# YuvalNirkin/hyperseg

Measured on AMD Instinct MI355X. Metric: frames/sec @ bs=1 HyperSeg-M 1024x512, higher is better.
Workload: dtype f32 storage and accumulation; level-4 inverted residual products as 3-term f16 splits (f32-class: 1.3e-7 of sum|a||b|; exact_f32 beside it)

## Files before the change

### hyperseg_amd/_hip.py

```python
import ctypes as C
import os
import types

import torch

_LIB_PATH = os.environ.get('HS_HIP_LIB') or os.path.join(os.path.dirname(os.path.abspath(__file__)), 'lib',
                                                         'libhyperseg_hip.so')

ACT_NONE, ACT_RELU, ACT_RELU6, ACT_SWISH = 0, 1, 2, 3
PAD_MODES = {'zeros': 0, 'reflect': 1, 'replicate': 2, 'circular': 3}
PREV_NONE, PREV_SAME, PREV_BILINEAR = 0, 1, 2

_STATUS = {-1: 'bad argument', -2: 'feature map does not tile into the weight grid (H % fh or W % fw != 0)',
           -3: 'unsupported shape', -4: 'tile does not fit the LDS'}


class HipLibraryError(RuntimeError):
    pass


class StageInputC(C.Structure):
    _fields_ = [('skip', C.c_void_p), ('prev', C.c_void_p),
                ('batch', C.c_int32), ('H', C.c_int32), ('W', C.c_int32),
                ('c_skip', C.c_int32), ('c_prev', C.c_int32),
# ... 33 lines not shown


class TtaPassC(C.Structure):
    _fields_ = [('x', C.c_void_p), ('Hi', C.c_int32), ('Wi', C.c_int32), ('Hm', C.c_int32), ('Wm', C.c_int32),
                ('flipped', C.c_int32), ('entry', C.c_int32)]


STATUS = 'hs_status'
i32, i64, vp = C.c_int32, C.c_int64, C.c_void_p
SIGNATURES = {
    'hs_version': ([], C.c_int),
    'hs_build_info': ([], C.c_char_p),
    'hs_signal2weights_fwd': ([vp, i32, i32, i32, i32, i32, i32, i32, vp, i32, i32, vp, i64, vp], STATUS),
    'hs_signal2weights_multi_fwd': ([vp, i32, i32, i32, i32, C.POINTER(S2wLayerC), i32, vp], STATUS),
    'hs_s2w_pack_floats': ([i32, i32, i32], C.c_int64),
    'hs_s2w_pack_fwd': ([vp, i32, i32, i32, vp, vp], STATUS),
    'hs_bank_pack_fwd': ([vp, i32, i32, i32, i32, i32, i32, vp, i64, vp], STATUS),
    'hs_bn_fold_fwd': ([vp, vp, vp, vp, C.c_float, i32, vp, vp, vp], STATUS),
    'hs_patch_conv_fwd': ([C.POINTER(StageInputC), i32, i32, vp, i64, i32, i32, i32, i32, i32,
                           C.POINTER(EpilogueC), vp, vp], STATUS),
    'hs_patch_conv_s2w_fwd': ([C.POINTER(StageInputC), i32, i32, vp, i64, i32, i32, C.POINTER(EpilogueC), vp,
                               vp, i32, i32, i32, i32, C.POINTER(S2wLayerC), i32, vp], STATUS),
    'hs_k1_chain_workspace': ([i32, i32, i32, C.POINTER(K1LevelC), i32], C.c_int64),
    'hs_k1_chain_fwd': ([i32, i32, i32, C.POINTER(K1LevelC), i32, vp, vp, vp], STATUS),
    'hs_decoder_chain_workspace': ([i32, i32, i32, C.POINTER(K1LevelC), i32, C.POINTER(ChainIrLevelC)], C.c_int64),
    'hs_decoder_chain_fwd': ([i32, i32, i32, C.POINTER(K1LevelC), i32, C.POINTER(ChainIrLevelC), vp, vp, vp], STATUS),
    'hs_meta_conv_fwd': ([vp, i32, i32, i32, i32, vp, i64] + [i32] * 13 + [C.POINTER(EpilogueC), vp, vp], STATUS),
    'hs_meta_conv_bwd': ([vp, i32, i32, i32, i32, vp, i64] + [i32] * 12 + [vp, vp, vp, i64, vp], STATUS),
    'hs_patch_conv_gen_fwd': ([C.POINTER(StageInputC), i32, i32, vp, i32, C.POINTER(S2wLayerC), i32,
                               C.POINTER(EpilogueC), vp, vp], STATUS),
    'hs_patch_ir_fwd': ([C.POINTER(StageInputC), i32, i32, vp, i64, i32, i32, C.POINTER(EpilogueC),
                         C.POINTER(EpilogueC), C.POINTER(EpilogueC), i32, i32, vp, vp], STATUS),
    'hs_patch_ir_v0_fwd': ([C.POINTER(StageInputC), i32, i32, vp, i64, i32, i32, C.POINTER(EpilogueC),
                            C.POINTER(EpilogueC), C.POINTER(EpilogueC), i32, vp, vp], STATUS),
    'hs_patch_ir_v0_ws_fwd': ([C.POINTER(StageInputC), i32, i32, vp, i64, i32, i32, C.POINTER(EpilogueC),
                               C.POINTER(EpilogueC), C.POINTER(EpilogueC), i32, vp, i64, vp, vp], STATUS),
    'hs_patch_ir_v0_workspace': ([C.POINTER(StageInputC), i32, i32, i32, i32], C.c_int64),
    'hs_halo_tiles_fwd': ([i32, vp, i32, i32, i32, i32, i32, i32, vp, i32, vp], STATUS),
    'hs_halo_tiles_bwd': ([i32, vp, i32, i32, i32, i32, i32, i32, vp, i32, vp], STATUS),
    'hs_tile_interior_fwd': ([i32, vp, i32, i32, i32, i32, i32, i32, vp, vp], STATUS),
    'hs_tile_interior_bwd': ([i32, vp, i32, i32, i32, i32, i32, i32, vp, vp], STATUS),
    'hs_dw_tiles_fwd': ([i32, vp, vp, i64, i32, i32, i32, i32, i32, i32, vp, i32, vp], STATUS),
    'hs_dw_tiles_bwd_in': ([i32, vp, vp, i64, i32, i32, i32, i32, i32, i32, vp, i32, vp], STATUS),
    'hs_dw_tiles_bwd_w': ([i32, vp, vp, i32, i32, i32, i32, i32, i32, vp, i64, i32, vp], STATUS),
    'hs_bank_unpack_fwd': ([vp, i64, i32, i32, i32, i32, i32, i32, vp, vp], STATUS),
    'hs_upsample_bilinear_bwd': ([vp, i64, i32, i32, i32, i32, i32, i32, vp, vp], STATUS),
    'hs_upsample_bilinear_bf16_fwd': ([vp, i32, i32, i32, i32, i32, i32, vp, vp], STATUS),
    'hs_upsample_bilinear_f16_fwd': ([vp, i32, i32, i32, i32, i32, i32, vp, vp], STATUS),
    'hs_upsample_bilinear_typed_bwd': ([i32, vp, i64, i32, i32, i32, i32, i32, i32, vp, vp], STATUS),
    'hs_bn_train_workspace': ([i32], C.c_int64),
    'hs_bn_train_stats_fwd': ([i32, vp, i32, i32, i64, vp, vp], STATUS),
    'hs_dw_tiles_bn_fwd': ([i32, vp, vp, vp, vp, vp, vp, C.c_float, C.c_float, i32, vp, vp, vp, vp, i64, i32, i32, i32, i32, i32, i32, vp, i32, vp], STATUS),
    'hs_dw_tiles_bn_bwd_w': ([i32, vp, vp, vp, vp, vp, vp, i32, i32, i32, i32, i32, i32, i32, vp, i64, i32, vp], STATUS),
    'hs_s2w_train_fwd': ([vp, i32, i32, i32, i32, C.POINTER(S2wTrainLayerC), i32, vp], STATUS),
    'hs_s2w_train_workspace': ([i32, i32, i32, C.POINTER(S2wTrainLayerC), i32], C.c_int64),
    'hs_s2w_train_bwd': ([vp, i32, i32, i32, i32, C.POINTER(S2wTrainLayerC), i32, vp, vp, i64, vp], STATUS),
    'hs_cross_entropy_fwd': ([vp, vp, i32, i32, i64, i64, vp, vp], STATUS),
    'hs_cross_entropy_bwd': ([vp, vp, i32, i32, i64, i64, vp, vp, vp], STATUS),
    'hs_cross_entropy_typed_fwd': ([i32, vp, vp, i32, i32, i64, i64, vp, vp], STATUS),
    'hs_cross_entropy_typed_bwd': ([i32, vp, vp, i32, i32, i64, i64, vp, vp, vp], STATUS),
    'hs_bootstrapped_ce_fwd': ([i32, vp, vp, i32, i32, i64, i64, i32, C.c_float, vp, vp, vp, vp, vp], STATUS),
    'hs_bootstrapped_ce_bwd': ([i32, vp, vp, i32, i32, i64, i64, vp, vp, vp, vp, vp], STATUS),
    'hs_cross_entropy_weighted_fwd': ([i32, vp, vp, vp, i32, i32, i64, i64, vp, vp], STATUS),
    'hs_cross_entropy_weighted_bwd': ([i32, vp, vp, vp, i32, i32, i64, i64, vp, vp, vp], STATUS),
    'hs_bootstrapped_ce_weighted_fwd': ([i32, vp, vp, vp, i32, i32, i64, i64, i32, C.c_float, vp, vp, vp, vp, vp], STATUS),
    'hs_bootstrapped_ce_weighted_bwd': ([i32, vp, vp, vp, i32, i32, i64, i64, vp, vp, vp, vp, vp], STATUS),
    'hs_bn_act_train_fwd': ([i32, vp, i32, i32, i64, vp, vp, vp, vp, C.c_float, C.c_float, i32, vp, vp, vp, vp, vp, vp], STATUS),
    'hs_bn_act_train_bwd': ([i32, vp, vp, i32, i32, i64, vp, vp, vp, vp, C.c_float, i32, vp, vp, vp, vp, vp], STATUS),
    'hs_dw_tiles_bn_bwd_in_partials': ([i32, i32, i32, i32, i32], C.c_int64),
    'hs_dw_tiles_bn_bwd_in': ([i32, vp, vp, i64, vp, vp, vp, vp, vp, i32, i32, i32, i32, i32, i32, i32, vp, vp, i32, vp], STATUS),
    'hs_bn_act_train_bwd_apply': ([i32, vp, vp, i32, i32, i64, vp, vp, vp, vp, i32, vp, i64, vp, vp, vp, vp], STATUS),
    'hs_bootstrap_mean_workspace': ([], C.c_int64),
    'hs_bootstrap_mean_fwd': ([vp, i32, i32, C.c_float, vp, vp, vp], STATUS),
    'hs_bootstrap_mean_bwd': ([vp, i32, vp, vp, vp, vp], STATUS),
    'hs_bootstrap_mean_batched_fwd': ([vp, i32, i32, i32, C.c_float, vp, vp, vp], STATUS),
    'hs_bootstrap_mean_batched_bwd': ([vp, i32, i32, vp, vp, vp, vp], STATUS),
    'hs_patch_ir_route': ([C.POINTER(StageInputC), i32, i32, i32, i32, i32, i32], C.c_int),
    'hs_patch_ir_form': ([C.POINTER(StageInputC), i32, i32, i64, i32, i32, i32, i32, i32, i32, C.POINTER(C.c_int32)], C.c_int),
    'hs_patch_ir_v0_route': ([C.POINTER(StageInputC), i32, i32, i64, i32, i32, i32, i32, C.POINTER(C.c_int32)], C.c_int),
    'hs_patch_conv_route': ([C.POINTER(StageInputC), i32, i32, i64] + [i32] * 10 + [C.POINTER(C.c_int32)], C.c_int),
    'hs_ir_tile_map': ([i32, i32, i32, C.POINTER(i32), C.POINTER(i32), C.POINTER(i32), i32], STATUS),
    'hs_upsample_bilinear_fwd': ([vp, i32, i32, i32, i32, i32, i32, vp, vp], STATUS),
    'hs_upsample_argmax_fwd': ([vp, i32, i32, i32, i32, i32, i32, vp, vp], STATUS),
    'hs_eval_max_classes': ([], C.c_int),
    'hs_upsample_confusion_fwd': ([vp, i32, i32, i32, i32, i32, i32, vp, i32, i32, i32, vp, vp, vp], STATUS),
    'hs_confusion_fwd': ([vp, i32, vp, i32, i32, i64, i32, i32, vp, vp], STATUS),
    'hs_upsample2_confusion_fwd': ([vp, i32, i32, i32, i32, i32, i32, i32, i32, vp, i32, i32, i32, vp, vp, vp], STATUS),
    'hs_tta_merge_fwd': ([C.POINTER(TtaPassC), i32, i32, i32, i32, vp, i32, i32, i32, i32, i32, vp, vp, vp, vp], STATUS),
    'hs_cross_entropy_score_fwd': ([i32, vp, vp, i32, i32, i64, i64, vp, i32, i32, vp, vp, vp], STATUS),
    'hs_upsample_ce_confusion_fwd': ([vp, i32, i32, i32, i32, i32, i32, vp, i32, i64, vp, i32, i32, vp, vp, vp], STATUS),
    'hs_cross_entropy_score_weighted_fwd': ([i32, vp, vp, vp, i32, i32, i64, i64, vp, i32, i32, vp, vp, vp], STATUS),
    'hs_upsample_ce_confusion_weighted_fwd': ([vp, i32, i32, i32, i32, i32, i32, vp, i32, vp, i64, vp, i32, i32, vp, vp, vp], STATUS),
    'hs_upsample2_ce_confusion_fwd': ([vp, i32, i32, i32, i32, i32, i32, i32, i32, vp, i32, i64, vp, i32, i32, vp, vp, vp], STATUS),
    'hs_upsample2_ce_confusion_weighted_fwd': ([vp, i32, i32, i32, i32, i32, i32, i32, i32, vp, i32, vp, i64, vp, i32, i32, vp, vp, vp], STATUS),
    'hs_stage_input_fwd': ([C.POINTER(StageInputC), vp, vp], STATUS),
    'hs_stage_input_typed_fwd': ([C.POINTER(StageInputC), i32, i32, vp, vp], STATUS),
    'hs_patch_conv_bwd_input': ([vp, vp, i64, i32, i32, i32, i32, i32, i32, i32, i32, i32, i32, i32, vp, vp], STATUS),
    'hs_patch_conv_bwd_weight': ([vp, vp, i32, i32, i32, i32, i32, i32, i32, i32, i32, i32, i32, vp, i64, vp], STATUS),
    'hs_patch_conv_bwd_route': ([i32, i32, i32, i32, i64] + [i32] * 11 + [C.POINTER(C.c_int32), C.POINTER(C.c_int32)], STATUS),
    'hs_patch_conv_plain_fwd': ([i32, vp, vp, i64, i32, i32, i32, i32, i32, i32, i32, i32, i32, i32, i32, vp, vp], STATUS),
    'hs_patch_conv_plain_bwd_in': ([i32, vp, vp, i64, i32, i32, i32, i32, i32, i32, i32, i32, i32, i32, i32, vp, vp], STATUS),
    'hs_patch_conv_plain_bwd_w': ([i32, vp, vp, i32, i32, i32, i32, i32, i32, i32, i32, i32, i32, i32, vp, i64, vp], STATUS),
    'hs_depthwise_conv_fwd': ([vp, i32, i32, i32, i32, vp, i32, i32, i32, i32, i32, i32, vp, vp, i32, vp, vp, vp, vp, vp], STATUS),
    'hs_pointwise_conv_fwd': ([vp, i32, i32, i32, vp, i32, vp, vp, vp, i32, vp, vp, vp], STATUS),
    'hs_affine_act_fwd': ([vp, i32, i32, i32, vp, vp, i32, vp, vp, vp], STATUS),
    'hs_patch_conv_bn_fwd': ([i32, vp, vp, vp, vp, vp, vp, C.c_float, C.c_float, i32, vp, vp, vp, vp, i64, i32, i32, i32, i32, i32, i32, i32, vp, vp], STATUS),
    'hs_patch_conv_bn_bwd_w': ([i32, vp, vp, vp, vp, vp, vp, i32, i32, i32, i32, i32, i32, i32, i32, vp, i64, vp], STATUS),
    'hs_bootstrap_mean_of_batch_fwd': ([vp, i32, i32, i32, C.c_float, vp, vp, vp, vp], STATUS),
    'hs_bootstrap_mean_of_batch_bwd': ([vp, i32, i32, vp, vp, vp, vp], STATUS),
    'hs_adam_blocks': ([vp, i32], C.c_int64),
    'hs_adam_step': ([vp, vp, vp, vp, vp, i32, vp, C.c_float, C.c_double, C.c_double, C.c_float, C.c_float, i32, i32, vp, vp], STATUS),
    'hs_adam_step_amp': ([vp, vp, vp, vp, vp, i32, vp, C.c_float, C.c_double, C.c_double, C.c_float, C.c_float, i32, i32, vp, vp, vp, vp], STATUS),
    'hs_depthwise_pool_blocks': ([i32, i32], C.c_int),
    'hs_depthwise_conv_se_fwd': ([vp, i32, i32, i32, i32, vp, i32, i32, i32, i32, i32, i32, vp, vp, i32, vp, vp, vp, C.POINTER(SeTailC), vp], STATUS),
    'hs_mbconv_expand_dw_se_fwd': ([vp, i32, i32, i32, i32, vp, i32, vp, vp, vp, i32, i32, i32, i32, i32, i32, vp, vp, vp, C.POINTER(SeTailC), vp], STATUS),
    'hs_se_tail_workspace': ([i32, i32, i32, i32, i64], C.c_int64),
    'hs_se_tail_tails': ([i32, i32, i32, i64], C.c_int),
    'hs_mbconv_se_workgroups': ([i32, i32, i32, i32, i32, i32], C.c_int64),
    'hs_stem_conv_fwd': ([vp, i32, i32, i32, i32, vp, i32, i32, i32, i32, i32, vp, vp, vp, vp], STATUS),
    'hs_mbconv_tiles': ([i32, i32, i32, i32], C.c_int),
    'hs_stem_dw_fwd': ([vp, i32, i32, i32, vp, i32, vp, vp, i32, i32, i32, i32, vp, i32, i32, i32, vp, vp, vp, vp, vp], STATUS),
    'hs_image_ingest_fwd': ([vp, i32, i32, i32, i32, i32, vp, vp, vp], STATUS),
    'hs_stem_dw_u8_fwd': ([vp, i32, vp, i32, i32, i32, vp, i32, vp, vp, i32, i32, i32, i32, vp, i32, i32, i32, vp, vp, vp, vp, vp], STATUS),
    'hs_overlay_fwd': ([vp, vp, i32, i32, i32, i32, vp, i32, i32, vp, vp], STATUS),
    'hs_upsample_overlay_fwd': ([vp, i32, i32, i32, i32, i32, i32, vp, i32, vp, i32, i32, vp, vp, vp], STATUS),
    'hs_upsample2_overlay_fwd': ([vp, i32, i32, i32, i32, i32, i32, i32, i32, vp, i32, vp, i32, i32, vp, vp, vp], STATUS),
    'hs_confidence_fwd': ([vp, i32, i32, i32, i32, i32, C.c_float, i32, vp, vp, vp], STATUS),
    'hs_upsample_confidence_fwd': ([vp, i32, i32, i32, i32, i32, i32, i32, C.c_float, i32, vp, vp, vp], STATUS),
    'hs_upsample2_confidence_fwd': ([vp, i32, i32, i32, i32, i32, i32, i32, i32, i32, C.c_float, i32, vp, vp, vp], STATUS),
    'hs_frame_resize_fwd': ([vp, i32, i32, i32, i32, vp, vp, i32, i32, vp, vp, i32, i32, i32, i32, i32, i32, i32, C.c_uint32, vp, vp, vp], STATUS),
    'hs_label_resize_fwd': ([vp, i32, i32, i32, i32, vp, i32, vp, i32, i32, i32, i32, i32, i32, i32, vp, i32, vp], STATUS),
    'hs_resize_tables_fwd': ([vp, i32, i32, i32, i32, i32, i32, i32, vp, vp, vp, vp, vp], STATUS),
    'hs_frame_resize_batch_fwd': ([vp, i32, i32, i32, i32, vp, vp, vp, vp, i32, i32, i32, C.c_uint32, vp, vp, vp], STATUS),
    'hs_label_resize_batch_fwd': ([vp, i32, i32, i32, i32, vp, vp, vp, i32, i32, i32, vp, i32, vp], STATUS),
    'hs_label_encode_fwd': ([vp, i32, i32, i32, i32, vp, i32, i32, i32, vp, i32, vp], STATUS),
    'hs_label_resize_coded_fwd': ([vp, i32, i32, i32, i32, vp, i32, vp, i32, i32, i32, i32, i32, i32, i32, vp, i32, i32, i32, vp, i32, vp], STATUS),
    'hs_label_resize_batch_coded_fwd': ([vp, i32, i32, i32, i32, vp, vp, vp, i32, i32, i32, vp, i32, i32, i32, vp, i32, vp], STATUS),
    'hs_color_jitter_fwd': ([vp, i32, i32, i32, i32, vp, vp, vp, vp, vp], STATUS),
    'hs_gaussian_blur_fwd': ([vp, i32, i32, i32, i32, vp, vp, vp, vp, vp, vp], STATUS),
    'hs_frame_rotate_fwd': ([vp, i32, i32, i32, i32, vp, i32, i32, C.c_uint32, C.c_uint32, vp, vp, vp], STATUS),
    'hs_label_rotate_fwd': ([vp, i32, i32, i32, i32, vp, i32, i32, i32, i32, vp, i32, vp], STATUS),
    'hs_resize_tables_ragged_fwd': ([vp, i32, i32, i32, i32, i32, i32, i32, vp, vp, vp, vp, vp], STATUS),
    'hs_color_jitter_ragged_fwd': ([vp, i32, i32, i32, i32, vp, vp, vp, vp, vp], STATUS),
    'hs_frame_resize_ragged_fwd': ([vp, i32, i32, i32, i32, vp, vp, vp, vp, i32, i32, i32, vp, vp], STATUS),
    'hs_label_resize_ragged_fwd': ([vp, i32, i32, i32, i32, vp, vp, vp, i32, i32, vp, vp], STATUS),
    'hs_frame_rotate_ragged_fwd': ([vp, i32, i32, i32, i32, vp, vp, vp, i32, i32, C.c_uint32, C.c_uint32, vp, vp, vp], STATUS),
    'hs_label_rotate_ragged_fwd': ([vp, i32, i32, i32, vp, vp, vp, i32, i32, i32, i32, vp, i32, vp], STATUS),
    'hs_mbconv_expand_dw_fwd': ([vp, i32, i32, i32, i32, vp, i32, vp, vp, vp, i32, i32, i32, i32, i32, i32, vp, vp, vp, vp, vp], STATUS),
    'hs_se_gate_fwd': ([vp, i32, i32, i32, C.c_float, vp, vp, i32, vp, vp, vp, vp, vp, i32, vp, vp, vp], STATUS),
    'hs_gemm_split_kp': ([i32], C.c_int),
    'hs_gemm_split_fwd': ([vp, vp, vp, vp, vp, i32, vp, vp, i32, i32, i32, i32, i32, vp], STATUS),
    'hs_gemm_split_se_fwd': ([vp, vp, vp, i32, C.c_float, vp, vp, i32, vp, vp, vp, vp, i32, vp, vp, i32, i32, i32, i32, i32, vp, vp, vp], STATUS),
    'hs_gemm_split_se_route': ([i32] * 6, C.c_int),
    'hs_gemm_split_conv2x2_fwd': ([vp, vp, vp, vp, i32, vp, vp, i32, i32, i32, i32, i32, i32, vp], STATUS),
    'hs_gemm_split_up2_fwd': ([vp, vp, vp, vp, i32, vp, i32, i32, i32, i32, i32, i32, vp], STATUS),
    'hs_depthwise_route': ([i32] * 11, C.c_int),
    'hs_mbconv_route': ([i32] * 11, C.c_int),
    'hs_stem_dw_route': ([i32] * 9, C.c_int),
    'hs_stem_route': ([i32] * 3, C.c_int),
    'hs_se_gate_route': ([i32] * 5, C.c_int),
    'hs_pointwise_route': ([i32] * 5, C.c_int),
    'hs_pooled_shift_fwd': ([vp, i32, C.c_float, vp, vp, vp, i32, i32, vp], STATUS),
}
EXPORTS = list(SIGNATURES)


def check(status, what):
    if status == 0:
        return
    if status < 0:
        raise HipLibraryError(f'{what}: {_STATUS.get(status, status)}')
    raise HipLibraryError(f'{what}: HIP launch failed with hipError_t {status}')


def _raise_unless_ok(status, fn, args):
    if status:
        check(status, fn.__name__)
    return status


def _load():
    if not os.path.exists(_LIB_PATH):
        raise HipLibraryError(
            f'{_LIB_PATH} is missing: build it with `python -m hyperseg_amd.build` (hipcc, gfx950). '
            'hyperseg_amd has no fallback path.')
    lib = C.CDLL(_LIB_PATH)
    run = types.SimpleNamespace()
    for name, (argtypes, returns) in SIGNATURES.items():
        fn = getattr(lib, name)
        fn.argtypes, fn.restype = argtypes, C.c_int if returns is STATUS else returns
        if returns is STATUS:
            checked = lib[name]
            checked.argtypes, checked.restype, checked.errcheck = argtypes, C.c_int, _raise_unless_ok
            setattr(run, name, checked)
    if lib.hs_version() != 1:
        raise HipLibraryError(f'ABI mismatch: library reports version {lib.hs_version()}, binding expects 1')
    return lib, run


lib, run = _load()


def ptr(t):
    return None if t is None else t.data_ptr()


def dev_ptr(t, name='tensor', dtype=torch.float32):
    if t is None:
        return None
    if not isinstance(t, torch.Tensor):
        raise TypeError(f'{name} must be a torch.Tensor')
    if not t.is_cuda:
        raise HipLibraryError(f'{name} is on {t.device}: the HyperSeg decoder path runs on an MI355X only '
                              '(hyperseg_amd has no CPU fallback)')
    if t.dtype != dtype:
        raise HipLibraryError(f'{name} must be {dtype}, got {t.dtype}')
    if not t.is_contiguous():
        raise HipLibraryError(f'{name} must be contiguous')
    return t.data_ptr()


class _NullScope:
    def __enter__(self):
        return None

    def __exit__(self, *exc):
        return False


_NULL_SCOPE = _NullScope()


def device_scope(device):
    if device.index is None or device.index == torch.cuda.current_device():
        return _NULL_SCOPE
    return torch.cuda.device(device)


def stream_ptr(device=None):
    return torch.cuda.current_stream(device).cuda_stream
```

### hyperseg_amd/csrc/hs_encoder.hip

```cpp
#include "hs_common.h"
#include "hs_se_tail.h"

namespace hs {

template <int K, int S, int PL, bool TILE, bool SET>
__global__ __launch_bounds__(256)
void depthwise_conv_kernel(const float* __restrict__ x, const float* __restrict__ w, const float* __restrict__ scale,
                           const float* __restrict__ shift, float* __restrict__ y, int C, int H, int W, int Ho, int Wo,
                           int pad_t, int pad_l, int act, float* __restrict__ pool_partial,
                           const float* __restrict__ in_scale, const float* __restrict__ in_shift, int nplanes, SeTail se) {
    const int plane = blockIdx.y + blockIdx.z * gridDim.y;
    if (plane >= nplanes) return;
    const int c = plane % C;
    unsigned se_gen = 0u;
    if constexpr (SET) se_gen = se.ws ? se_tag(se, plane / C) : 0u;
    const bool pre = in_scale != nullptr;
    float isc = 1.0f, ish = 0.0f;
    if constexpr (TILE) {
        if (pre) { isc = in_scale[c]; ish = in_shift[c]; }
    }
    const int wq = (Wo + 3) >> 2;
    const int q = blockIdx.x * blockDim.x + threadIdx.x;
    const bool live = q < Ho * wq;
    float psum = 0.0f;
// ... 463 lines not shown
                                 const hs_se_tail* se_in, void* stream) {
    if ((in_scale != nullptr) != (in_shift != nullptr)) return HS_ERR_BAD_ARG;
    if (!x || !w || !y || batch <= 0 || channels <= 0 || H <= 0 || W <= 0 || Ho <= 0 || Wo <= 0) return HS_ERR_BAD_ARG;
    if (pad_t < 0 || pad_l < 0 || (scale && !shift)) return HS_ERR_BAD_ARG;
    const long nplanes = (long)batch * channels;
    if (nplanes > 65535L * 65535L) return HS_ERR_UNSUPPORTED;
    const int quads = Ho * ((Wo + 3) / 4);
    const int threads = depthwise_threads(Ho, Wo);
    const int gy = nplanes > 65535 ? 32768 : (int)nplanes;
    dim3 grid((quads + threads - 1) / threads, gy, (unsigned)((nplanes + gy - 1) / gy));
    hipStream_t s = (hipStream_t)stream;
    SeTail se{};
    if (se_in) {
        const int st = make_se_tail(se_in, batch, channels, (int)grid.x, (long)channels * grid.x, Ho * Wo, se);
        if (st != HS_OK) return st;
    }
    const size_t se_lds = se_in ? (size_t)se_lds_floats(se.Csq) * sizeof(float) : 0;
#define HS_DW_(KK, SS, PP, SETV) hipLaunchKernelGGL((depthwise_conv_kernel<KK, SS, PP, false, SETV>), grid, dim3(threads), se_lds, s, x, w, scale, shift, \
                                             y, channels, H, W, Ho, Wo, pad_t, pad_l, act, pool_partial, in_scale, in_shift, (int)nplanes, se)
#define HS_DW(KK, SS, PP) do { if (se_in) HS_DW_(KK, SS, PP, true); else HS_DW_(KK, SS, PP, false); } while (0)
    const int route = depthwise_route(nplanes, k, stride, pad_l, W, Ho, Wo, (((size_t)x) & 15) == 0, in_scale != nullptr);
    if (route < 0) return route;
    if ((route >> 8) == HS_DW_FORM_TILED) {
        const size_t tile_lds = depthwise_tile_lds(k, stride, Wo);
        const size_t lds = tile_lds > se_lds ? tile_lds : se_lds;
#define HS_DWT_(KK, SS, SETV) hipLaunchKernelGGL((depthwise_conv_kernel<KK, SS, -1, true, SETV>), grid, dim3(threads), lds, s, x, w, scale, shift, y, \
                                          channels, H, W, Ho, Wo, pad_t, pad_l, act, pool_partial, in_scale, in_shift, (int)nplanes, se)
#define HS_DWT(KK, SS) do { if (se_in) HS_DWT_(KK, SS, true); else HS_DWT_(KK, SS, false); } while (0)
        if (k == 3 && stride == 1) HS_DWT(3, 1); else if (k == 3) HS_DWT(3, 2); else if (stride == 1) HS_DWT(5, 1); else HS_DWT(5, 2);
#undef HS_DWT
#undef HS_DWT_
        return launch_status();
    }
    switch (route) {
        case HS_DW_ROUTE(HS_DW_FORM_VECTOR, 3, 1, 1): HS_DW(3, 1, 1); break;
        case HS_DW_ROUTE(HS_DW_FORM_GENERIC, 3, 1, 0): HS_DW(3, 1, -1); break;
        case HS_DW_ROUTE(HS_DW_FORM_VECTOR, 3, 2, 0): HS_DW(3, 2, 0); break;
        case HS_DW_ROUTE(HS_DW_FORM_VECTOR, 3, 2, 1): HS_DW(3, 2, 1); break;
        case HS_DW_ROUTE(HS_DW_FORM_GENERIC, 3, 2, 0): HS_DW(3, 2, -1); break;
        case HS_DW_ROUTE(HS_DW_FORM_VECTOR, 5, 1, 2): HS_DW(5, 1, 2); break;
        case HS_DW_ROUTE(HS_DW_FORM_GENERIC, 5, 1, 0): HS_DW(5, 1, -1); break;
        case HS_DW_ROUTE(HS_DW_FORM_VECTOR, 5, 2, 1): HS_DW(5, 2, 1); break;
        case HS_DW_ROUTE(HS_DW_FORM_VECTOR, 5, 2, 2): HS_DW(5, 2, 2); break;
        case HS_DW_ROUTE(HS_DW_FORM_GENERIC, 5, 2, 0): HS_DW(5, 2, -1); break;
        default: return HS_ERR_UNSUPPORTED;
    }
#undef HS_DW
#undef HS_DW_
    return launch_status();
}

extern "C" int hs_depthwise_route(int32_t batch, int32_t channels, int32_t H, int32_t W, int32_t k, int32_t stride, int32_t pad_l,
                                  int32_t Ho, int32_t Wo, int32_t x_aligned16, int32_t prologue) {
    if (batch <= 0 || channels <= 0 || H <= 0 || W <= 0 || Ho <= 0 || Wo <= 0 || pad_l < 0) return HS_ERR_BAD_ARG;
    if ((long)batch * channels > 65535L * 65535L) return HS_ERR_UNSUPPORTED;
    return depthwise_route((long)batch * channels, k, stride, pad_l, W, Ho, Wo, x_aligned16 != 0, prologue != 0);
}

extern "C" int hs_depthwise_conv_fwd(const float* x, int32_t batch, int32_t channels, int32_t H, int32_t W,
                                     const float* w, int32_t k, int32_t stride, int32_t pad_t, int32_t pad_l,
                                     int32_t Ho, int32_t Wo, const float* scale, const float* shift, int32_t act,
                                     float* y, float* pool_partial, const float* in_scale, const float* in_shift,
                                     void* stream) {
    return depthwise_conv_launch(x, batch, channels, H, W, w, k, stride, pad_t, pad_l, Ho, Wo, scale, shift, act, y, pool_partial,
                                 in_scale, in_shift, nullptr, stream);
}

extern "C" int hs_depthwise_conv_se_fwd(const float* x, int32_t batch, int32_t channels, int32_t H, int32_t W,
                                        const float* w, int32_t k, int32_t stride, int32_t pad_t, int32_t pad_l,
                                        int32_t Ho, int32_t Wo, const float* scale, const float* shift, int32_t act,
                                        float* y, const float* in_scale, const float* in_shift, const hs_se_tail* se,
                                        void* stream) {
    if (!se) return HS_ERR_BAD_ARG;
    return depthwise_conv_launch(x, batch, channels, H, W, w, k, stride, pad_t, pad_l, Ho, Wo, scale, shift, act, y, nullptr,
                                 in_scale, in_shift, se, stream);
}

extern "C" int64_t hs_se_tail_workspace(int32_t batch, int32_t channels, int32_t c_squeezed, int32_t nblk, int64_t wgs_per_batch) {
    int T, L;
    if (batch <= 0 || !se_tail_plan(channels, c_squeezed, nblk, wgs_per_batch, T, L)) return 0;
    SeTail t{};
    t.B = batch; t.C = channels; t.Csq = c_squeezed; t.nblk = nblk; t.T = T; t.L = L;
    return (int64_t)(se_ws_words(t) * sizeof(se_u64));
}

extern "C" int hs_se_tail_tails(int32_t channels, int32_t c_squeezed, int32_t nblk, int64_t wgs_per_batch) {
    int T, L;
    return se_tail_plan(channels, c_squeezed, nblk, wgs_per_batch, T, L) ? T : 0;
}

extern "C" int hs_depthwise_pool_blocks(int32_t Ho, int32_t Wo) {
    const int quads = Ho * ((Wo + 3) / 4);
    const int threads = quads >= 256 ? 256 : ((quads + 63) / 64) * 64;
    return (quads + threads - 1) / threads;
}

static int se_early_fold(int nblk) { return nblk <= 256 ? 1 : (nblk <= 512 ? 2 : 4); }

static int se_gate_route(int channels, int nblk, int c_squeezed, bool proj, bool aligned16) {
    const long units = (long)channels * ((nblk & 3) == 0 ? nblk >> 2 : nblk);
    if ((channels & 3) == 0 && channels <= 768 && c_squeezed <= SEF_MAX_CSQ && units <= 2048) return HS_SE_ROUTE_FUSED;
    static const bool off = [] { const char* e = getenv("HS_SE_EARLY"); return e && atoi(e) == 0; }();
    const int fold = se_early_fold(nblk);
    if (!off && !proj && (channels & 3) == 0 && channels * fold <= 4 * SEE_MAX_IT && c_squeezed <= 8 && (nblk & (4 * fold - 1)) == 0 &&
        nblk <= 1024 && aligned16) return HS_SE_ROUTE_EARLY;
    if (HS_SE_FUSED_WIDE && (channels & 3) == 0 && channels <= 256 && c_squeezed <= SEF_MAX_CSQ && units <= 6144) return HS_SE_ROUTE_FUSED_WIDE;
    return HS_SE_ROUTE_TWO_LAUNCH;
}

extern "C" int hs_se_gate_route(int32_t channels, int32_t nblk, int32_t c_squeezed, int32_t with_w_proj, int32_t aligned16) {
    if (channels <= 0 || nblk <= 0 || c_squeezed <= 0) return HS_ERR_BAD_ARG;
    if (c_squeezed > 65535) return HS_ERR_UNSUPPORTED;
    return se_gate_route(channels, nblk, c_squeezed, with_w_proj != 0, aligned16 != 0);
}

extern "C" int hs_se_gate_fwd(const float* partial, int32_t batch, int32_t channels, int32_t nblk, float inv_hw,
                              const float* w_reduce, const float* b_reduce, int32_t c_squeezed, const float* w_expand,
                              const float* b_expand, float* squeezed, float* gate, const float* w_proj, int32_t c_out,
                              const float* out_scale, float* w_scaled, void* stream) {
    if (!partial || !w_reduce || !b_reduce || !w_expand || !b_expand || !squeezed || !gate || batch <= 0 || channels <= 0 ||
        nblk <= 0 || c_squeezed <= 0) return HS_ERR_BAD_ARG;
    if ((w_proj != nullptr) != (w_scaled != nullptr) || (w_proj && c_out <= 0) || (out_scale && !w_proj)) return HS_ERR_BAD_ARG;
    if (batch > 65535 || c_squeezed > 65535) return HS_ERR_UNSUPPORTED;
    hipStream_t s = (hipStream_t)stream;
    const int row_groups = w_proj ? (c_out + 63) / 64 : 1;
    const int route = se_gate_route(channels, nblk, c_squeezed, w_proj != nullptr, (((size_t)partial | (size_t)w_reduce) & 15) == 0);
    if (route == HS_SE_ROUTE_FUSED) {
        hipLaunchKernelGGL((se_gate_fused_kernel<8, 3>), dim3((channels + 63) / 64, batch, row_groups), dim3(256), 0, s, partial, nblk,
                           inv_hw, w_reduce, b_reduce, w_expand, b_expand, channels, c_squeezed, squeezed, gate, w_proj, c_out,
                           out_scale, w_scaled);
        return launch_status();
    }
    if (route == HS_SE_ROUTE_EARLY) {
        const int fold = se_early_fold(nblk);
        hipLaunchKernelGGL(se_gate_early_kernel, dim3(1, batch), dim3(256), 0, s, partial, nblk / fold, inv_hw, w_reduce, b_reduce, w_expand,
                           b_expand, channels * fold, c_squeezed, squeezed, gate, fold);
        return launch_status();
    }
    if (route == HS_SE_ROUTE_FUSED_WIDE) {
        hipLaunchKernelGGL((se_gate_fused_kernel<24, 1>), dim3((channels + 63) / 64, batch, row_groups), dim3(256), 0, s, partial, nblk,
                           inv_hw, w_reduce, b_reduce, w_expand, b_expand, channels, c_squeezed, squeezed, gate, w_proj, c_out,
                           out_scale, w_scaled);
        return launch_status();
    }
    hipLaunchKernelGGL(se_squeeze_kernel, dim3(c_squeezed, batch), dim3(256), 0, s, partial, nblk, inv_hw, w_reduce,
                       b_reduce, channels, c_squeezed, squeezed);
    int st = launch_status();
    if (st != HS_OK) return st;
    hipLaunchKernelGGL(se_excite_kernel, dim3((channels + 63) / 64, batch, row_groups), dim3(256), 0, s, squeezed, w_expand,
                       b_expand, channels, c_squeezed, gate, w_proj, c_out, out_scale, w_scaled);
    return launch_status();
}

namespace hs {

using f32x4 = __attribute__((ext_vector_type(4))) float;

template <int NB, int NT, bool VEC = false>
__global__ __launch_bounds__(256)
void pointwise_conv_kernel(const float* __restrict__ x, const float* __restrict__ w, const float* __restrict__ gate,
                           const float* __restrict__ scale, const float* __restrict__ shift,
                           const float* __restrict__ residual, float* __restrict__ y, int Cin, int Cout, int P, int act) {
    const int lane = threadIdx.x & 63, wave = threadIdx.x >> 6;
    const int lrow = lane & 15, lk = lane >> 4;
    const int b = blockIdx.z;
    const int o0 = blockIdx.y * 32;
    const int p0 = (blockIdx.x * 4 + wave) * (16 * NT);
    if (p0 >= P) return;
    const float* __restrict__ xb = x + (size_t)b * Cin * P;
    const float* __restrict__ gb = gate ? gate + (size_t)b * Cin : nullptr;
    f32x4 acc[2][NT];
#pragma unroll
    for (int m = 0; m < 2; ++m)
#pragma unroll
        for (int n = 0; n < NT; ++n) acc[m][n] = f32x4{0.f, 0.f, 0.f, 0.f};
    int orow[2]; bool ook[2];
#pragma unroll
    for (int m = 0; m < 2; ++m) { const int o = o0 + 16 * m + lrow; ook[m] = o < Cout; orow[m] = ook[m] ? o : Cout - 1; }
    int pcol[NT]; bool pok[NT];
#pragma unroll
    for (int n = 0; n < NT; ++n) { const int p = VEC ? p0 + 4 * lrow + n : p0 + 16 * n + lrow; pok[n] = p < P; pcol[n] = pok[n] ? p : P - 1; }
    static_assert(!VEC || NT == 4, "interleaved tiles: four pixels per lane");
    constexpr int KU = 4;
    float av[2][KU][2], bv[2][KU][NT];
    auto load_batch = [&](int i, float (&a)[KU][2], float (&bb)[KU][NT]) {
#pragma unroll
        for (int u = 0; u < KU; ++u) {
            const int k = i * 4 * KU + 4 * u + lk;
            const bool kok = k < Cin;
            const int kc = kok ? k : Cin - 1;
            const float g = (gb ? gb[kc] : 1.0f) * (kok ? 1.0f : 0.0f);
#pragma unroll
            for (int m = 0; m < 2; ++m) a[u][m] = w[(size_t)orow[m] * Cin + kc] * (ook[m] ? 1.0f : 0.0f);
            if constexpr (VEC) {
                const f32x4 v = *reinterpret_cast<const f32x4*>(xb + (size_t)kc * P + pcol[0]);
#pragma unroll
                for (int n = 0; n < NT; ++n) bb[u][n] = v[n] * g;
            } else {
#pragma unroll
                for (int n = 0; n < NT; ++n) bb[u][n] = xb[(size_t)kc * P + pcol[n]] * g;
            }
        }
    };
    load_batch(0, av[0], bv[0]);
    float scv[2][4], shv[2][4];
#pragma unroll
    for (int m = 0; m < 2; ++m)
#pragma unroll
        for (int r = 0; r < 4; ++r) {
            const int o = min(o0 + 16 * m + 4 * lk + r, Cout - 1);
            scv[m][r] = scale ? scale[o] : 1.0f;
            shv[m][r] = shift ? shift[o] : 0.0f;
        }
    float rv[2][4][NT];
    if (residual) {
#pragma unroll
        for (int m = 0; m < 2; ++m)
#pragma unroll
            for (int r = 0; r < 4; ++r) {
                const int o = min(o0 + 16 * m + 4 * lk + r, Cout - 1);
                if constexpr (VEC) {
                    const f32x4 v = *reinterpret_cast<const f32x4*>(residual + ((size_t)b * Cout + o) * P + pcol[0]);
#pragma unroll
                    for (int n = 0; n < NT; ++n) rv[m][r][n] = v[n];
                } else {
#pragma unroll
                    for (int n = 0; n < NT; ++n) rv[m][r][n] = residual[((size_t)b * Cout + o) * P + pcol[n]];
                }
            }
    } else {
#pragma unroll
        for (int m = 0; m < 2; ++m)
#pragma unroll
            for (int r = 0; r < 4; ++r)
#pragma unroll
                for (int n = 0; n < NT; ++n) rv[m][r][n] = 0.0f;
    }
#pragma unroll
    for (int i = 0; i < NB; ++i) {
        if (i + 1 < NB) load_batch(i + 1, av[(i + 1) & 1], bv[(i + 1) & 1]);
#pragma unroll
        for (int u = 0; u < KU; ++u)
#pragma unroll
            for (int m = 0; m < 2; ++m)
#pragma unroll
                for (int n = 0; n < NT; ++n)
                    acc[m][n] = __builtin_amdgcn_mfma_f32_16x16x4f32(av[i & 1][u][m], bv[i & 1][u][n], acc[m][n], 0, 0, 0);
    }
#pragma unroll
    for (int m = 0; m < 2; ++m)
#pragma unroll
        for (int r = 0; r < 4; ++r) {
            const int o = o0 + 16 * m + 4 * lk + r;
            if (o >= Cout) continue;
            float ov[NT];
#pragma unroll
            for (int n = 0; n < NT; ++n) {
                float v = fmaf(acc[m][n][r], scv[m][r], shv[m][r]);
                if (act == 3) v = swishf(v);
                else v = apply_act(v, act);
                ov[n] = v + rv[m][r][n];
            }
            if constexpr (VEC) {
                *reinterpret_cast<f32x4*>(y + ((size_t)b * Cout + o) * P + pcol[0]) = f32x4{ov[0], ov[1], ov[2], ov[3]};
            } else {
#pragma unroll
                for (int n = 0; n < NT; ++n)
                    if (pok[n]) y[((size_t)b * Cout + o) * P + pcol[n]] = ov[n];
            }
        }
}

template <int NB>
static int launch_pointwise(int nt, bool vec, dim3 grid, hipStream_t s, const float* x, const float* w, const float* gate,
                            const float* scale, const float* shift, const float* residual, float* y, int c_in, int c_out,
                            int pixels, int act) {
#define HS_PW(NT) hipLaunchKernelGGL((pointwise_conv_kernel<NB, NT>), grid, dim3(256), 0, s, x, w, gate, scale, shift, \
                                     residual, y, c_in, c_out, pixels, act)
    if (vec) hipLaunchKernelGGL((pointwise_conv_kernel<NB, 4, true>), grid, dim3(256), 0, s, x, w, gate, scale, shift, residual, y, c_in,
                                c_out, pixels, act);
    else if (nt == 4) HS_PW(4); else if (nt == 2) HS_PW(2); else HS_PW(1);
#undef HS_PW
    return launch_status();
}

}

static int pointwise_route(int batch, int c_in, int c_out, int pixels, bool aligned16) {
    if (batch > 65535 || (c_out + 31) / 32 > 65535) return HS_ERR_UNSUPPORTED;
    if (c_in > 128) return HS_ERR_UNSUPPORTED;
    const int mblocks = (c_out + 31) / 32;
    int nt = 4;
    while (nt > 1 && (long)((pixels + 64 * nt - 1) / (64 * nt)) * mblocks * batch < 512) nt >>= 1;
    static const bool vec_off = [] { const char* e = getenv("HS_PW_VEC"); return e && atoi(e) == 0; }();
    const bool vec = !vec_off && nt == 4 && (pixels & 63) == 0 && aligned16;
    const int nb = (c_in + 15) / 16;
    return HS_PW_ROUTE(nb, nt, vec ? 1 : 0);
}

extern "C" int hs_pointwise_route(int32_t batch, int32_t c_in, int32_t c_out, int32_t pixels, int32_t aligned16) {
    if (batch <= 0 || c_in <= 0 || c_out <= 0 || pixels <= 0) return HS_ERR_BAD_ARG;
    return pointwise_route(batch, c_in, c_out, pixels, aligned16 != 0);
}

extern "C" int hs_pointwise_conv_fwd(const float* x, int32_t batch, int32_t c_in, int32_t pixels, const float* w,
                                     int32_t c_out, const float* gate, const float* scale, const float* shift, int32_t act,
// ... 171 lines not shown
```

### hyperseg_amd/csrc/hs_gemm_split.hip

```cpp
#include "hs_common.h"
#include "hs_se_gate_phases.h"
#include <type_traits>

namespace hs {

using half8 = __attribute__((ext_vector_type(8))) _Float16;
using gs_f32x4 = __attribute__((ext_vector_type(4))) float;

__device__ __forceinline__ int gs_exp_of(float m) { return min(max(__float_as_int(m) >> 23, 27), 254); }
__device__ __forceinline__ float gs_scale_of(int eb) { return __int_as_float((268 - eb) << 23); }
__device__ __forceinline__ float gs_inv_scale_of(int eb) { return __int_as_float((eb - 14) << 23); }

struct GemmSplitArgs {
    const _Float16* __restrict__ wf;
    const float* __restrict__ w_inv;
    const float* __restrict__ gate; const float* __restrict__ x;
    const float* shift;
    const float* residual;
    float* y;
    int M, K, KST, N, act;
    int conv_wo;
    float* pool_partial;
    int up2_wo;
};

struct GemmSeArgs {
    const float* __restrict__ partial;
    const float* __restrict__ w1; const float* __restrict__ b1;
    const float* __restrict__ w2t; const float* __restrict__ b2;
    float* gate_out; float* squeezed_out;
    float inv_hw; int nblk, Csq;
};
template <bool SEG> struct GemmSeOperand {};
template <> struct GemmSeOperand<true> : GemmSeArgs {};

#ifndef HS_GS_NARROW_MAX_WG
#define HS_GS_NARROW_MAX_WG 128
#endif

#ifndef HS_GS_TALL_MIN_WG
#define HS_GS_TALL_MIN_WG 257
#endif

template <int KS, int NWV, bool FAST, int NS, int MT, int NCH, bool PATCH, bool SEG = false>
__global__ __launch_bounds__(64 * NWV)
void gemm_split_kernel(GemmSplitArgs a, GemmSeOperand<SEG> se) {
    static_assert(!SEG || (FAST && !PATCH && NCH == 1 && (NWV == 8 ? KS <= 3 : KS == 1)), "SEG: the project convolutions' forms only");
    extern __shared__ __attribute__((aligned(16))) float gs_red[];
    constexpr int nthr = 64 * NWV, nwv = NWV;
    constexpr int NP = 16 * NS, NR = 16 * MT, NE = NR * NP;
    const int tid = threadIdx.x, lane = tid & 63, wave = tid >> 6;
    const int lrow = lane & 15, kg = lane >> 4;
    const int n0 = blockIdx.x * NP, r0 = blockIdx.y * MT, b = blockIdx.z;
    const float* __restrict__ xb = a.x + (size_t)b * a.K * a.N;
    const float* __restrict__ gb = a.gate ? a.gate + (size_t)b * a.K : nullptr;
    float* yb = a.y + (size_t)b * a.M * a.N * (a.up2_wo > 0 ? 4 : 1);
    const float* rb = a.residual ? a.residual + (size_t)b * a.M * a.N : nullptr;
    const int rt_max = (a.M + 15) >> 4;

    using gs_f32x2 = __attribute__((ext_vector_type(2))) float;
    const int ncol0 = min(n0 + NS * lrow, a.N - (FAST && !PATCH && NS == 2 ? 2 : 1)), ncol1 = min(n0 + NS * lrow + 1, a.N - 1);
    float xv[NCH][NS][KS][8];
    if constexpr (PATCH) {
        const int oy = ncol0 / a.conv_wo, ox = ncol0 - oy * a.conv_wo;
        const float* __restrict__ win = xb + (size_t)(2 * oy) * (2 * a.conv_wo) + 2 * ox;
        const int cmax = (a.K >> 2) - 1;
#pragma unroll
        for (int c = 0; c < NCH; ++c)
#pragma unroll
            for (int s = 0; s < KS; ++s)
#pragma unroll
                for (int q = 0; q < 4; ++q) {
                    const int ch = min((((wave * NCH + c) * KS + s) * 32 + 8 * kg) / 4 + (q >> 1), cmax);
                    const float* src = win + (size_t)ch * (4 * a.N) + (q & 1) * (2 * a.conv_wo);
                    if constexpr (NS == 1) {
                        const gs_f32x2 v = *reinterpret_cast<const gs_f32x2*>(src);
                        xv[c][0][s][2 * q] = v[0]; xv[c][0][s][2 * q + 1] = v[1];
                    } else {
                        const gs_f32x4 v = *reinterpret_cast<const gs_f32x4*>(src);
                        xv[c][0][s][2 * q] = v[0]; xv[c][0][s][2 * q + 1] = v[1];
                        xv[c][1][s][2 * q] = v[2]; xv[c][1][s][2 * q + 1] = v[3];
                    }
                }
    } else {
#pragma unroll
        for (int c = 0; c < NCH; ++c)
#pragma unroll
            for (int s = 0; s < KS; ++s)
#pragma unroll
                for (int j = 0; j < 8; ++j) {
                    const int k = ((wave * NCH + c) * KS + s) * 32 + 8 * kg + j;
                    const int kc = min(k, a.K - 1);
                    if constexpr (NS == 1) {
                        xv[c][0][s][j] = xb[(size_t)kc * a.N + ncol0];
                    } else if constexpr (FAST) {
                        const gs_f32x2 v = *reinterpret_cast<const gs_f32x2*>(xb + (size_t)kc * a.N + ncol0);
                        xv[c][0][s][j] = v[0]; xv[c][1][s][j] = v[1];
                    } else {
                        xv[c][0][s][j] = xb[(size_t)kc * a.N + ncol0]; xv[c][1][s][j] = xb[(size_t)kc * a.N + ncol1];
                    }
                }
    }
    constexpr int NG = PATCH ? 1 : NCH;
    float gv[NG][KS][8];
    if constexpr (!PATCH) {
#pragma unroll
        for (int c = 0; c < NCH; ++c)
#pragma unroll
            for (int s = 0; s < KS; ++s) {
                const int k0 = ((wave * NCH + c) * KS + s) * 32 + 8 * kg;
                if constexpr (SEG) {
                } else if constexpr (FAST) {
                    const float* gp = gb ? gb + min(k0, a.K - 8) : a.w_inv;
                    const gs_f32x4 g0 = *reinterpret_cast<const gs_f32x4*>(gp), g1 = *reinterpret_cast<const gs_f32x4*>(gp + 4);
#pragma unroll
                    for (int j = 0; j < 4; ++j) { gv[c][s][j] = g0[j]; gv[c][s][4 + j] = g1[j]; }
                } else {
#pragma unroll
                    for (int j = 0; j < 8; ++j) gv[c][s][j] = gb ? gb[min(k0 + j, a.K - 1)] : 1.0f;
                }
            }
    }
    half8 ah[2][KS], al[2][KS];
    auto load_a = [&](int q) {
        const int rt = min(r0 + q % MT, rt_max - 1);
#pragma unroll
        for (int s = 0; s < KS; ++s) {
            const _Float16* blk = a.wf + ((size_t)(rt * a.KST + (wave * NCH + q / MT) * KS + s) * 2) * 512 + lane * 8;
            ah[q & 1][s] = *reinterpret_cast<const half8*>(blk);
            al[q & 1][s] = *reinterpret_cast<const half8*>(blk + 512);
        }
    };
    load_a(0);
    constexpr int TE = (NE + nthr - 1) / nthr;
    float wi[TE], sh[TE], yo[TE];
    auto load_tail = [&]() {
#pragma unroll
        for (int i = 0; i < TE; ++i) {
            const int e = min(tid + i * nthr, NE - 1);
            const int row = min(16 * r0 + e / NP, a.M - 1), col = min(n0 + (e & (NP - 1)), a.N - 1);
            wi[i] = a.w_inv[min(16 * r0 + e / NP, 16 * rt_max - 1)];
            sh[i] = a.shift ? a.shift[row] : 0.0f;
            yo[i] = rb ? rb[(size_t)row * a.N + col] : 0.0f;
        }
    };
    constexpr bool LATE_TAIL = KS * NCH >= 3;
    if constexpr (!LATE_TAIL) load_tail();
    constexpr int SE_PV = SEP_MAX_UNITS / nthr, SE_RW = SEP_MAX_CSQ / NWV, SE_W1U = NWV == 8 ? (KS < 3 ? KS : 3) : 1;
    constexpr int SE_CI = NWV == 8 && KS >= 3 ? 2 : 1;
    float4 se_pv[SE_PV], se_w1v[SE_RW][SE_W1U];
    float se_b1v[SE_RW], se_w2q[SE_CI][4][8], se_b2v[SE_CI];
    if constexpr (SEG) {
        se_load_units<nthr, SE_PV>(se.partial + (size_t)b * a.K * se.nblk, se.nblk, a.K, tid, se_pv);
        se_load_reduce<NWV, SE_RW, SE_W1U>(se.w1, se.b1, a.K, se.Csq, wave, lane, se_w1v, se_b1v);
#pragma unroll
        for (int ci = 0; ci < SE_CI; ++ci) se_load_expand(se.w2t, se.b2, a.K, se.Csq, min(tid + nthr * ci, a.K - 1), se_w2q[ci], se_b2v[ci]);
    }
    __builtin_amdgcn_sched_barrier(0);
    if constexpr (SEG) {
        float* mean_c = gs_red + SEP_MEAN; float* zs = gs_red + SEP_ZS; float* gate_s = gs_red + SEP_GATE;
        se_channel_means<nthr, SE_PV>(se_pv, se.nblk, a.K, se.inv_hw, tid, gs_red + SEP_PART, mean_c);
        se_squeeze_rows<NWV, SE_RW, SE_W1U>(se_w1v, se_b1v, mean_c, a.K, se.Csq, wave, lane, zs);
        __syncthreads();
        const bool first = blockIdx.x == 0 && blockIdx.y == 0;
        if (first && se.squeezed_out && tid < se.Csq) se.squeezed_out[(size_t)b * se.Csq + tid] = zs[tid];
#pragma unroll
        for (int ci = 0; ci < SE_CI; ++ci) {
            const int ch = tid + nthr * ci;
            const float g = se_channel_gate(se_w2q[ci], se_b2v[ci], zs, se.Csq);
            if (ch < a.K) {
                gate_s[ch] = g;
                if (first && se.gate_out) se.gate_out[(size_t)b * a.K + ch] = g;
            }
        }
        __syncthreads();
#pragma unroll
        for (int s = 0; s < KS; ++s) {
            const float* gp = gate_s + min((wave * KS + s) * 32 + 8 * kg, a.K - 8);
            const gs_f32x4 g0 = *reinterpret_cast<const gs_f32x4*>(gp), g1 = *reinterpret_cast<const gs_f32x4*>(gp + 4);
#pragma unroll
            for (int j = 0; j < 4; ++j) { gv[0][s][j] = g0[j]; gv[0][s][4 + j] = g1[j]; }
        }
        __syncthreads();
    }

    gs_f32x4 tot[MT][NS];
#pragma unroll
    for (int c = 0; c < NCH; ++c) {
        float invb[NS];
        half8 bh[NS][KS], bl[NS][KS];
#pragma unroll
        for (int t = 0; t < NS; ++t) {
            unsigned mx = 0;
#pragma unroll
            for (int s = 0; s < KS; ++s) {
                const int k0 = ((wave * NCH + c) * KS + s) * 32 + 8 * kg;
#pragma unroll
                for (int j = 0; j < 8; ++j) {
                    const float mk = (FAST || PATCH ? k0 : k0 + j) < a.K ? 1.0f : 0.0f;
                    float g = mk;
                    if constexpr (!PATCH) g = SEG || gb ? gv[c][s][j] * mk : mk;
                    xv[c][t][s][j] *= g;
                    mx = max(mx, __float_as_uint(xv[c][t][s][j]) & 0x7fffffffu);
                }
            }
            {
                auto r16 = __builtin_amdgcn_permlane16_swap(mx, mx, false, false);
                mx = max(r16[0], r16[1]);
                auto r32 = __builtin_amdgcn_permlane32_swap(mx, mx, false, false);
                mx = max(r32[0], r32[1]);
            }
            const int eb = gs_exp_of(__uint_as_float(mx));
            const float sc = gs_scale_of(eb);
            invb[t] = gs_inv_scale_of(eb);
#pragma unroll
            for (int s = 0; s < KS; ++s) {
                if constexpr (FAST || PATCH) {
                    unsigned hh[4], ll[4];
#pragma unroll
                    for (int j = 0; j < 4; ++j) {
                        asm("v_fma_mixlo_f16 %0, %2, %4, 0\n\t"
                            "v_fma_mixhi_f16 %0, %3, %4, 0\n\t"
                            "v_fma_mixlo_f16 %1, %2, %4, -%0 op_sel_hi:[0,0,1]\n\t"
                            "v_fma_mixhi_f16 %1, %3, %4, -%0 op_sel:[0,0,1] op_sel_hi:[0,0,1]"
                            : "=&v"(hh[j]), "=&v"(ll[j]) : "v"(xv[c][t][s][2 * j]), "v"(xv[c][t][s][2 * j + 1]), "v"(sc));
                    }
                    using gs_u32x4 = __attribute__((ext_vector_type(4))) unsigned;
                    bh[t][s] = __builtin_bit_cast(half8, gs_u32x4{hh[0], hh[1], hh[2], hh[3]});
                    bl[t][s] = __builtin_bit_cast(half8, gs_u32x4{ll[0], ll[1], ll[2], ll[3]});
                } else {
#pragma unroll
                    for (int j = 0; j < 8; ++j) {
                        const float v = xv[c][t][s][j] * sc;
                        const _Float16 hi = (_Float16)v;
                        bh[t][s][j] = hi;
                        bl[t][s][j] = (_Float16)(v - (float)hi);
                    }
                }
            }
        }
        if (c == 0) {
            load_a(1);
            if constexpr (LATE_TAIL) load_tail();
        }
        __builtin_amdgcn_sched_barrier(0);
#pragma unroll
        for (int mt = 0; mt < MT; ++mt) {
            const int q = c * MT + mt;
            gs_f32x4 acc[NS];
#pragma unroll
            for (int t = 0; t < NS; ++t) {
                acc[t] = gs_f32x4{0.f, 0.f, 0.f, 0.f};
#pragma unroll
                for (int s = 0; s < KS; ++s) {
                    acc[t] = __builtin_amdgcn_mfma_f32_16x16x32_f16(al[q & 1][s], bh[t][s], acc[t], 0, 0, 0);
                    acc[t] = __builtin_amdgcn_mfma_f32_16x16x32_f16(ah[q & 1][s], bl[t][s], acc[t], 0, 0, 0);
                    acc[t] = __builtin_amdgcn_mfma_f32_16x16x32_f16(ah[q & 1][s], bh[t][s], acc[t], 0, 0, 0);
                }
            }
            if (q + 2 < NCH * MT) { load_a(q + 2); __builtin_amdgcn_sched_barrier(0); }
#pragma unroll
            for (int t = 0; t < NS; ++t) {
#pragma unroll
                for (int r = 0; r < 4; ++r) {
                    const float v = c == 0 ? acc[t][r] * invb[t] : fmaf(acc[t][r], invb[t], tot[mt][t][r]);
                    if (c == NCH - 1) gs_red[(wave * NR + 16 * mt + 4 * kg + r) * NP + NS * lrow + t] = v;
                    else tot[mt][t][r] = v;
                }
            }
        }
    }
    __syncthreads();
    auto tail = [&](auto act_kind) {
        constexpr int ACT = decltype(act_kind)::value;
#pragma unroll
        for (int i = 0; i < TE; ++i) {
            const int e = tid + i * nthr;
            if (e < NE) {
                const int row = 16 * r0 + e / NP, col = n0 + (e & (NP - 1));
                float t = 0.0f;
#pragma unroll
                for (int w = 0; w < nwv; ++w) t += gs_red[w * NE + e];
                const bool live = row < a.M && col < a.N;
                float v = fmaf(t, wi[i], sh[i]);
                if constexpr (ACT == HS_ACT_SWISH) v = swishf(v);
                else if constexpr (ACT == HS_ACT_RELU) v = fmaxf(v, 0.0f);
                else if constexpr (ACT == HS_ACT_RELU6) v = fminf(fmaxf(v, 0.0f), 6.0f);
                v += yo[i];
                if (live) {
                    if (a.up2_wo > 0) {
                        const int oy = col / a.up2_wo, ox = col - oy * a.up2_wo;
                        float* dst = yb + (size_t)row * (4 * a.N) + (size_t)(2 * oy) * (2 * a.up2_wo) + 2 * ox;
                        *reinterpret_cast<gs_f32x2*>(dst) = gs_f32x2{v, v};
                        *reinterpret_cast<gs_f32x2*>(dst + 2 * a.up2_wo) = gs_f32x2{v, v};
                    } else {
                        yb[(size_t)row * a.N + col] = v;
                    }
                }
                if constexpr (NP == 16) {
                    if (a.pool_partial) {
                        const float rs = rowsum16(live ? v : 0.0f);
                        if ((e & 15) == 0 && row < a.M) a.pool_partial[((size_t)b * a.M + row) * gridDim.x + blockIdx.x] = rs;
                    }
                }
            }
        }
    };
    if (a.act == HS_ACT_SWISH) tail(std::integral_constant<int, HS_ACT_SWISH>{});
    else if (a.act == HS_ACT_NONE) tail(std::integral_constant<int, HS_ACT_NONE>{});
    else if (a.act == HS_ACT_RELU) tail(std::integral_constant<int, HS_ACT_RELU>{});
    else tail(std::integral_constant<int, HS_ACT_RELU6>{});
}

__global__ __launch_bounds__(256)
void pooled_shift_kernel(const float* __restrict__ partial, int nblk, float inv_p, const float* __restrict__ wb,
                         const float* __restrict__ shift, float* __restrict__ out, int M, int C) {
    extern __shared__ float ps_mean[];
    const int tid = threadIdx.x, lane = tid & 63, wave = tid >> 6;
    for (int c = tid; c < C; c += 256) {
        float t = 0.0f;
        for (int j = 0; j < nblk; ++j) t += partial[(size_t)c * nblk + j];
        ps_mean[c] = t * inv_p;
    }
    __syncthreads();
    const int r0 = 16 * blockIdx.x + 4 * wave;
    float acc[4] = {0.f, 0.f, 0.f, 0.f};
#pragma unroll 2
    for (int c = lane; c < C; c += 64) {
        const float m = ps_mean[c];
#pragma unroll
        for (int i = 0; i < 4; ++i) acc[i] = fmaf(wb[(size_t)min(r0 + i, M - 1) * C + c], m, acc[i]);
    }
#pragma unroll
    for (int i = 0; i < 4; ++i) {
        const float t = wave_sum64(acc[i]);
        if (lane == 0 && r0 + i < M) out[r0 + i] = shift[r0 + i] + t;
    }
}

static bool gemm_split_plan(int K, int& nwv, int& ks, int& nch) {
    const int steps = (K + 31) / 32;
    nwv = 2;
    while (nwv < 8 && nwv < steps) nwv *= 2;
    const int per = (steps + nwv - 1) / nwv;
    nch = per > 5 ? 2 : 1;
    ks = (steps + nwv * nch - 1) / (nwv * nch);
    return ks <= 5;
}

}

using namespace hs;

extern "C" int hs_gemm_split_kp(int32_t c_in) {
    int nwv, ks, nch;
    if (c_in <= 0 || !gemm_split_plan(c_in, nwv, ks, nch)) return HS_ERR_UNSUPPORTED;
    return nwv * nch * ks * 32;
}

struct GemmSplitPolicy {
    int nwv, ks, nch;
    bool narrow, tall, fast;
    dim3 grid;
    size_t lds;
};
static int gemm_split_policy(int batch, int c_out, int c_in, int kp, int pixels, GemmSplitPolicy& p) {
    if (!gemm_split_plan(c_in, p.nwv, p.ks, p.nch)) return HS_ERR_UNSUPPORTED;
    if (kp != p.nwv * p.nch * p.ks * 32 || (p.ks > 1 && p.nwv != 8)) return HS_ERR_BAD_ARG;
    if (batch > 65535 || (c_out + 31) / 32 > 65535) return HS_ERR_UNSUPPORTED;
    p.grid = dim3((pixels + 31) / 32, ((c_out + 15) / 16 + 1) / 2, batch);
    const size_t wgs = (size_t)p.grid.x * p.grid.y * p.grid.z;
    p.narrow = wgs <= HS_GS_NARROW_MAX_WG && pixels > 16;
    p.tall = wgs >= HS_GS_TALL_MIN_WG && c_out > 32;
    if (p.narrow) p.grid.x = (pixels + 15) / 16;
    if (p.tall) p.grid.y = ((c_out + 15) / 16 + 3) / 4;
    p.lds = (size_t)p.nwv * (p.narrow ? 512 : p.tall ? 2048 : 1024) * sizeof(float);
    p.fast = (c_in & 7) == 0 && (pixels & 1) == 0 && c_in >= 8;
    return HS_OK;
}

static int launch_gemm_split_plain(const void* w_frag, const float* w_inv, const float* gate, const float* x, const float* shift,
                                   int32_t act, const float* residual, float* y, int32_t batch, int32_t c_out, int32_t c_in,
                                   int32_t kp, int32_t pixels, int up2_wo, void* stream) {
    if (!w_frag || !w_inv || !x || !y || batch <= 0 || c_out <= 0 || c_in <= 0 || pixels <= 0) return HS_ERR_BAD_ARG;
    if (act < 0 || act > 3) return HS_ERR_BAD_ARG;
    GemmSplitPolicy pol;
    const int pst = gemm_split_policy(batch, c_out, c_in, kp, pixels, pol);
    if (pst != HS_OK) return pst;
    const int nwv = pol.nwv, ks = pol.ks, nch = pol.nch;
    const bool narrow = pol.narrow, tall = pol.tall, fast = pol.fast;
    dim3 grid = pol.grid;
    const size_t lds = pol.lds;
    GemmSplitArgs a{(const _Float16*)w_frag, w_inv, gate, x, shift, residual, y, c_out, c_in, kp / 32, pixels, act, 0, nullptr, up2_wo};
    hipStream_t s = (hipStream_t)stream;
#define HS_GS_(KSV, NWV, F) do { \
        if (narrow) hipLaunchKernelGGL((gemm_split_kernel<KSV, NWV, F, 1, 2, 1, false>), grid, dim3(64 * NWV), lds, s, a, GemmSeOperand<false>{}); \
        else if (tall) hipLaunchKernelGGL((gemm_split_kernel<KSV, NWV, F, 2, 4, 1, false>), grid, dim3(64 * NWV), lds, s, a, GemmSeOperand<false>{}); \
        else hipLaunchKernelGGL((gemm_split_kernel<KSV, NWV, F, 2, 2, 1, false>), grid, dim3(64 * NWV), lds, s, a, GemmSeOperand<false>{}); } while (0)
#define HS_GS(KSV, NWV) do { if (fast) HS_GS_(KSV, NWV, true); else HS_GS_(KSV, NWV, false); } while (0)
    if (nch == 2) {
        if (!fast || up2_wo > 0) return HS_ERR_UNSUPPORTED;
        grid.x = (pixels + 15) / 16; grid.y = ((c_out + 15) / 16 + 1) / 2;
        const size_t lds2 = (size_t)8 * 512 * sizeof(float);
#define HS_GS2(KSV) hipLaunchKernelGGL((gemm_split_kernel<KSV, 8, true, 1, 2, 2, false>), grid, dim3(512), lds2, s, a, GemmSeOperand<false>{})
        switch (ks) { case 3: HS_GS2(3); break; case 4: HS_GS2(4); break; case 5: HS_GS2(5); break; default: return HS_ERR_UNSUPPORTED; }
#undef HS_GS2
        return launch_status();
    }
    switch (ks) {
        case 1: if (nwv == 2) HS_GS(1, 2); else if (nwv == 4) HS_GS(1, 4); else HS_GS(1, 8); break;
        case 2: HS_GS(2, 8); break;
        case 3: HS_GS(3, 8); break;
        case 4: HS_GS(4, 8); break;
        default: HS_GS(5, 8); break;
    }
#undef HS_GS
#undef HS_GS_
    return launch_status();
}

static int gemm_split_se_route(int channels, int nblk, int c_squeezed, int c_out, int pixels, bool aligned16, int batch, GemmSplitPolicy& pol) {
    if (channels <= 0 || nblk <= 0 || c_squeezed <= 0 || c_out <= 0 || pixels <= 0 || batch <= 0) return HS_ERR_BAD_ARG;
    const int kp = hs_gemm_split_kp(channels);
    if (kp < 0) return HS_ERR_UNSUPPORTED;
    const int pst = gemm_split_policy(batch, c_out, channels, kp, pixels, pol);
    if (pst != HS_OK) return pst;
    if (hs_se_gate_route(channels, nblk, c_squeezed, 0, aligned16 ? 1 : 0) != HS_SE_ROUTE_FUSED) return HS_ERR_UNSUPPORTED;
    if (!aligned16 || !pol.fast || pol.nch != 1 || channels > SEP_MAX_C || c_squeezed > SEP_MAX_CSQ) return HS_ERR_UNSUPPORTED;
    if (pol.ks > (pol.nwv == 8 ? 3 : 1)) return HS_ERR_UNSUPPORTED;
    return HS_GSE_ROUTE(pol.ks, pol.nwv);
}

extern "C" int hs_gemm_split_se_route(int32_t channels, int32_t nblk, int32_t c_squeezed, int32_t c_out, int32_t pixels, int32_t aligned16) {
    GemmSplitPolicy pol;
    return gemm_split_se_route(channels, nblk, c_squeezed, c_out, pixels, aligned16 != 0, 1, pol);
}

extern "C" int hs_gemm_split_se_fwd(const void* w_frag, const float* w_inv, const float* partial, int32_t nblk, float inv_hw,
                                    const float* w_reduce, const float* b_reduce, int32_t c_squeezed, const float* w_expand_t,
                                    const float* b_expand, const float* x, const float* shift, int32_t act, const float* residual,
                                    float* y, int32_t batch, int32_t c_out, int32_t c_in, int32_t kp, int32_t pixels,
                                    float* gate_out, float* squeezed_out, void* stream) {
    if (!w_frag || !w_inv || !x || !y || batch <= 0 || c_out <= 0 || c_in <= 0 || pixels <= 0) return HS_ERR_BAD_ARG;
    if (!partial || !w_reduce || !b_reduce || !w_expand_t || !b_expand || nblk <= 0 || c_squeezed <= 0) return HS_ERR_BAD_ARG;
    if (act < 0 || act > 3) return HS_ERR_BAD_ARG;
    GemmSplitPolicy pol;
    const bool aligned16 = (((size_t)partial | (size_t)w_reduce) & 15) == 0;
    const int route = gemm_split_se_route(c_in, nblk, c_squeezed, c_out, pixels, aligned16, batch, pol);
    if (route < 0) return route;
    if (kp != pol.nwv * pol.ks * 32) return HS_ERR_BAD_ARG;
    GemmSplitArgs a{(const _Float16*)w_frag, w_inv, nullptr, x, shift, residual, y, c_out, c_in, kp / 32, pixels, act, 0, nullptr, 0};
    GemmSeOperand<true> se{{partial, w_reduce, b_reduce, w_expand_t, b_expand, gate_out, squeezed_out, inv_hw, nblk, c_squeezed}};
    const size_t se_lds = (size_t)SEP_LDS_FLOATS * sizeof(float);
    const size_t lds = pol.lds > se_lds ? pol.lds : se_lds;
    hipStream_t s = (hipStream_t)stream;
#define HS_GSE(KSV, NWV) do { \
        if (pol.narrow) hipLaunchKernelGGL((gemm_split_kernel<KSV, NWV, true, 1, 2, 1, false, true>), pol.grid, dim3(64 * NWV), lds, s, a, se); \
        else if (pol.tall) hipLaunchKernelGGL((gemm_split_kernel<KSV, NWV, true, 2, 4, 1, false, true>), pol.grid, dim3(64 * NWV), lds, s, a, se); \
        else hipLaunchKernelGGL((gemm_split_kernel<KSV, NWV, true, 2, 2, 1, false, true>), pol.grid, dim3(64 * NWV), lds, s, a, se); } while (0)
    switch (pol.ks) {
        case 1: if (pol.nwv == 2) HS_GSE(1, 2); else if (pol.nwv == 4) HS_GSE(1, 4); else HS_GSE(1, 8); break;
        case 2: HS_GSE(2, 8); break;
        default: HS_GSE(3, 8); break;
    }
#undef HS_GSE
    return launch_status();
}

extern "C" int hs_gemm_split_fwd(const void* w_frag, const float* w_inv, const float* gate, const float* x,
                                 const float* shift, int32_t act, const float* residual, float* y,
                                 int32_t batch, int32_t c_out, int32_t c_in, int32_t kp, int32_t pixels, void* stream) {
    return launch_gemm_split_plain(w_frag, w_inv, gate, x, shift, act, residual, y, batch, c_out, c_in, kp, pixels, 0, stream);
}

extern "C" int hs_gemm_split_up2_fwd(const void* w_frag, const float* w_inv, const float* x, const float* shift, int32_t act,
                                     float* y, int32_t batch, int32_t c_out, int32_t c_in, int32_t kp, int32_t Ho, int32_t Wo,
                                     void* stream) {
    if (Ho <= 0 || Wo <= 0 || (((size_t)y) & 7) != 0) return HS_ERR_BAD_ARG;
    return launch_gemm_split_plain(w_frag, w_inv, nullptr, x, shift, act, nullptr, y, batch, c_out, c_in, kp, Ho * Wo, Wo, stream);
}

extern "C" int hs_pooled_shift_fwd(const float* partial, int32_t nblk, float inv_pixels, const float* wb, const float* shift,
                                   float* shift_out, int32_t rows, int32_t channels, void* stream) {
    if (!partial || !wb || !shift || !shift_out || nblk <= 0 || rows <= 0 || channels <= 0) return HS_ERR_BAD_ARG;
    if (channels > 8192) return HS_ERR_UNSUPPORTED;
    hipLaunchKernelGGL(pooled_shift_kernel, dim3((rows + 15) / 16), dim3(256), (size_t)channels * sizeof(float), (hipStream_t)stream,
                       partial, nblk, inv_pixels, wb, shift, shift_out, rows, channels);
    return launch_status();
}

extern "C" int hs_gemm_split_conv2x2_fwd(const void* w_frag, const float* w_inv, const float* x, const float* shift, int32_t act,
                                         float* y, float* pool_partial, int32_t batch, int32_t c_out, int32_t c_in, int32_t kp,
                                         int32_t Ho, int32_t Wo, void* stream) {
    if (!w_frag || !w_inv || !x || !y || batch <= 0 || c_out <= 0 || c_in <= 0 || Ho <= 0 || Wo <= 0) return HS_ERR_BAD_ARG;
    if (act < 0 || act > 3) return HS_ERR_BAD_ARG;
    int nwv, ks, nch;
    if (c_in > (1 << 20) || !gemm_split_plan(4 * c_in, nwv, ks, nch) || nwv != 8 || (Wo & 1) || (c_in & 1)) return HS_ERR_UNSUPPORTED;
    if (kp != nwv * nch * ks * 32) return HS_ERR_BAD_ARG;
    if ((((size_t)x) & 15) != 0) return HS_ERR_BAD_ARG;
    const int pixels = Ho * Wo;
    if (batch > 65535 || (c_out + 31) / 32 > 65535) return HS_ERR_UNSUPPORTED;
    GemmSplitArgs a{(const _Float16*)w_frag, w_inv, nullptr, x, shift, nullptr, y, c_out, 4 * c_in, kp / 32, pixels, act, Wo, pool_partial, 0};
    dim3 grid((pixels + 15) / 16, ((c_out + 15) / 16 + 1) / 2, batch);
    const size_t lds = (size_t)8 * 512 * sizeof(float);
    hipStream_t s = (hipStream_t)stream;
#define HS_GP(KSV, NCHV) hipLaunchKernelGGL((gemm_split_kernel<KSV, 8, true, 1, 2, NCHV, true>), grid, dim3(512), lds, s, a, GemmSeOperand<false>{})
    switch (ks * 2 + nch - 1) {
        case 2: HS_GP(1, 1); break;
        case 4: HS_GP(2, 1); break;
        case 6: HS_GP(3, 1); break;
        case 8: HS_GP(4, 1); break;
        case 10: HS_GP(5, 1); break;
        case 7: HS_GP(3, 2); break;
        case 9: HS_GP(4, 2); break;
        case 11: HS_GP(5, 2); break;
        default: return HS_ERR_UNSUPPORTED;
    }
#undef HS_GP
    return launch_status();
}
```

### hyperseg_amd/csrc/hs_se_gate_phases.h

```cpp
#pragma once
#include "hs_common.h"

namespace hs {

constexpr int SEP_MAX_C = 768, SEP_MAX_CSQ = 32, SEP_MAX_UNITS = 2048;
constexpr int SEP_MEAN = 0, SEP_ZS = SEP_MEAN + SEP_MAX_C, SEP_GATE = SEP_ZS + SEP_MAX_CSQ, SEP_PART = SEP_GATE + SEP_MAX_C;
constexpr int SEP_LDS_FLOATS = SEP_PART + SEP_MAX_UNITS + SEP_MAX_C;

template <int NTHR, int PV>
__device__ __forceinline__ void se_load_units(const float* __restrict__ pb, int nblk, int C, int tid, float4 (&pv)[PV]) {
    const bool vec = (nblk & 3) == 0;
    const int units = C * (vec ? nblk >> 2 : nblk);
    if (vec) {
#pragma unroll
        for (int k = 0; k < PV; ++k) pv[k] = reinterpret_cast<const float4*>(pb)[min(tid + NTHR * k, units - 1)];
    } else {
#pragma unroll
        for (int k = 0; k < PV; ++k) pv[k] = make_float4(pb[min(tid + NTHR * k, units - 1)], 0.0f, 0.0f, 0.0f);
    }
}

template <int NTHR, int PV>
__device__ __forceinline__ void se_channel_means(const float4 (&pv)[PV], int nblk, int C, float inv_hw, int tid, float* part, float* mean) {
    const int qn = (nblk & 3) == 0 ? nblk >> 2 : nblk, units = C * qn;
#pragma unroll
    for (int k = 0; k < PV; ++k) {
        const int e = tid + NTHR * k;
        if (e < units) {
            const int ch = e / qn;
            part[ch * (qn + 1) + (e - ch * qn)] = (pv[k].x + pv[k].y) + (pv[k].z + pv[k].w);
        }
    }
    __syncthreads();
    for (int ch = tid; ch < C; ch += NTHR) {
        const float* run = part + ch * (qn + 1);
        float t = 0.0f;
        for (int i = 0; i < qn; ++i) t += run[i];
        mean[ch] = t * inv_hw;
    }
    __syncthreads();
}

template <int NWV, int RW, int W1U>
__device__ __forceinline__ void se_load_reduce(const float* __restrict__ w1, const float* __restrict__ b1, int C, int Csq, int wave, int lane,
                                               float4 (&w1v)[RW][W1U], float (&b1v)[RW]) {
    const int c4 = C >> 2;
#pragma unroll
    for (int r = 0; r < RW; ++r) {
        const int j = min(wave + NWV * r, Csq - 1);
        b1v[r] = b1[j];
#pragma unroll
        for (int u = 0; u < W1U; ++u) {
            w1v[r][u] = make_float4(0.0f, 0.0f, 0.0f, 0.0f);
            if (NWV * r < Csq && 64 * u < c4)
                w1v[r][u] = reinterpret_cast<const float4*>(w1 + (size_t)j * C)[min(lane + 64 * u, c4 - 1)];
        }
    }
}

template <int NWV, int RW, int W1U>
__device__ __forceinline__ void se_squeeze_rows(const float4 (&w1v)[RW][W1U], const float (&b1v)[RW], const float* mean, int C, int Csq,
                                                int wave, int lane, float* zs) {
    const int c4 = C >> 2;
    float4 mv[W1U];
#pragma unroll
    for (int u = 0; u < W1U; ++u) {
        const int k = lane + 64 * u;
        mv[u] = *reinterpret_cast<const float4*>(mean + 4 * min(k, c4 - 1));
        if (k >= c4) mv[u] = make_float4(0.0f, 0.0f, 0.0f, 0.0f);
    }
#pragma unroll
    for (int r = 0; r < RW; ++r) {
        if (NWV * r < Csq) {
            float a = 0.0f;
#pragma unroll
            for (int u = 0; u < W1U; ++u) {
                a = fmaf(w1v[r][u].x, mv[u].x, a); a = fmaf(w1v[r][u].y, mv[u].y, a);
                a = fmaf(w1v[r][u].z, mv[u].z, a); a = fmaf(w1v[r][u].w, mv[u].w, a);
            }
            a = wave_sum64(a);
            const int j = wave + NWV * r;
            if (lane == 0 && j < Csq) zs[j] = swishf(a + b1v[r]);
        }
    }
}

__device__ __forceinline__ void se_load_expand(const float* __restrict__ w2t, const float* __restrict__ b2, int C, int Csq, int c,
                                               float (&w2q)[4][8], float& b2v) {
    const int jq = (Csq + 3) >> 2;
#pragma unroll
    for (int i = 0; i < 4; ++i)
#pragma unroll
        for (int u = 0; u < 8; ++u) w2q[i][u] = w2t[(size_t)min(i * jq + u, Csq - 1) * C + c];
    b2v = b2[c];
}

__device__ __forceinline__ float se_channel_gate(const float (&w2q)[4][8], float b2v, const float* zs, int Csq) {
    const int jq = (Csq + 3) >> 2;
    float q[4];
#pragma unroll
    for (int i = 0; i < 4; ++i) {
        const int j0 = i * jq, j1 = min(j0 + jq, Csq);
        float acc = 0.0f;
#pragma unroll
        for (int u = 0; u < 8; ++u)
            if (j0 + u < j1) acc = fmaf(w2q[i][u], zs[min(j0 + u, SEP_MAX_CSQ - 1)], acc);
        q[i] = acc;
    }
    return sigmoidf_fast(((q[0] + q[1]) + (q[2] + q[3])) + b2v);
}

}
```

### hyperseg_amd/functional.py

```python
import collections
import ctypes as C
import functools
import os
import threading

import torch

from . import _hip
from ._hip import ACT_NONE, ACT_RELU, ACT_RELU6, PAD_MODES

BN_EPS_DEFAULT = 1e-5
DTYPE_CODES = {torch.float32: 0, torch.bfloat16: 1, torch.float16: 2}
S2W_TRAIN_MAX_LAYERS = 8
COSCHEDULE_BANKS = os.environ.get('HS_COSCHEDULE_BANKS', '0') == '1'


def _round_up(n, m):
    return (n + m - 1) // m * m


def _device_of(a):
    if isinstance(a, torch.Tensor):
        return a.device
    if isinstance(a, (StageInput, BankRef, SignalRef, U8Frame)):
# ... 1025 lines not shown
        return None
    if code < 0:
        _hip.check(code, what)
    return code


_DW_FORMS = {0: 'generic', 1: 'vector', 2: 'tiled'}
_MB_FORMS = {0: 'full', 1: 'lean', 2: 'stem'}
SE_ROUTES = {0: 'fused', 1: 'early', 2: 'fused_wide', 3: 'two_launch'}


def depthwise_route(shape, k, stride, pad_left, out_size, prologue=False, aligned=True):
    b, c, h, w = shape
    r = _route(_hip.lib.hs_depthwise_route(b, c, h, w, k, stride, pad_left, out_size[0], out_size[1], int(bool(aligned)), int(bool(prologue))),
               'hs_depthwise_route')
    if r is None:
        return None
    form, name = _DW_FORMS[r >> 8], f'k{(r >> 4) & 15}s{(r >> 2) & 3}'
    return f'{form}_{name}_pl{r & 3}' if form == 'vector' else f'{form}_{name}'


def mbconv_route(shape, c_mid, k, stride, out_size, aligned=True, se_tail=False):
    b, cin, h, w = shape
    r = _route(_hip.lib.hs_mbconv_route(b, cin, h, w, c_mid, k, stride, out_size[0], out_size[1], int(bool(aligned)), int(bool(se_tail))),
               'hs_mbconv_route')
    return None if r is None else f'{_MB_FORMS[r >> 8]}_k{(r >> 4) & 15}s{r & 15}'


def stem_dw_route(size, c_mid, stem_pad_top, stem_pad_left, stem_out_size, k=3, aligned=True):
    r = _route(_hip.lib.hs_stem_dw_route(size[0], size[1], c_mid, stem_pad_top, stem_pad_left, stem_out_size[0], stem_out_size[1], k,
                                         int(bool(aligned))), 'hs_stem_dw_route')
    return None if r is None else f'{_MB_FORMS[r >> 8]}_k{(r >> 4) & 15}s{r & 15}'


def se_gate_route(channels, nblk, c_squeezed, w_proj=False, aligned=True):
    r = _route(_hip.lib.hs_se_gate_route(channels, nblk, c_squeezed, int(bool(w_proj)), int(bool(aligned))), 'hs_se_gate_route')
    return None if r is None else SE_ROUTES[r]


STEM_ROUTES = {0: 'generic', 1: 'vector_pl0', 2: 'vector_pl1'}


def stem_route(width, pad_left, aligned=True):
    return STEM_ROUTES[_route(_hip.lib.hs_stem_route(width, pad_left, int(bool(aligned))), 'hs_stem_route')]


def pointwise_route(batch, c_in, c_out, pixels, aligned=True):
    r = _route(_hip.lib.hs_pointwise_route(batch, c_in, c_out, pixels, int(bool(aligned))), 'hs_pointwise_route')
    if r is None:
        return None
    return f'vec_nb{r >> 8}' if r & 1 else f'nt{(r >> 4) & 15}_nb{r >> 8}'


class SplitWeights:
    __slots__ = ('frag', 'inv', 'c_out', 'c_in', 'kp')

    def __init__(self, frag, inv, c_out, c_in, kp):
        self.frag, self.inv, self.c_out, self.c_in, self.kp = frag, inv, c_out, c_in, kp


@torch.no_grad()
def gemm_split_weights(w, row_scale=None, max_k=1280):
    w = w.detach().flatten(1).float()
    m, k = w.shape
    kp = _hip.lib.hs_gemm_split_kp(k) if k <= max_k else -1
    if kp < 0:
        return None
    if row_scale is not None:
        w = w * row_scale.detach().float()[:, None]
    eb = (w.abs().amax(1).contiguous().view(torch.int32) >> 23).clamp(27, 254)
    one = torch.ones(m, device=w.device)
    ws = w * torch.ldexp(one, 141 - eb)[:, None]
    hi = ws.half()
    lo = (ws - hi.float()).half()
    rt = -(-m // 16)
    pad = (0, kp - k, 0, 16 * rt - m)
    hi, lo = torch.nn.functional.pad(hi, pad), torch.nn.functional.pad(lo, pad)
    inv = torch.nn.functional.pad(torch.ldexp(one, eb - 141), (0, 16 * rt - m), value=1.0)

    def fragment_order(t):
        return t.view(rt, 16, kp // 32, 4, 8).permute(0, 2, 3, 1, 4)
    frag = torch.stack([fragment_order(hi), fragment_order(lo)], dim=2).contiguous()
    return SplitWeights(frag, inv.contiguous(), m, k, kp)


@_on_operand_device
def gemm_split(sw, x, gate=None, shift=None, act=ACT_NONE, residual=None, out=None):
    b, cin, h, w = x.shape
    if cin != sw.c_in:
        raise ValueError(f'input has {cin} channels, the weight {sw.c_in}')
    shape = (b, sw.c_out, h, w)
    if out is None:
        out = torch.empty(shape, device=x.device, dtype=torch.float32)
    elif tuple(out.shape) != shape:
        raise ValueError(f'out has shape {tuple(out.shape)}, expected {shape}')
    if residual is not None and tuple(residual.shape) != shape:
        raise ValueError(f'residual has shape {tuple(residual.shape)}, expected {shape}')
    if gate is not None and tuple(gate.shape) != (b, cin):
        raise ValueError(f'gate has shape {tuple(gate.shape)}, expected {(b, cin)}')
    if shift is not None and shift.numel() != sw.c_out:
        raise ValueError(f'shift has {shift.numel()} entries, expected {sw.c_out}')
    _hip.run.hs_gemm_split_fwd(_hip.dev_ptr(sw.frag, 'w_frag', torch.float16), _hip.dev_ptr(sw.inv, 'w_inv'),
                               _hip.dev_ptr(gate, 'gate') if gate is not None else None, _hip.dev_ptr(x, 'x'),
                               _hip.dev_ptr(shift, 'shift') if shift is not None else None, int(act),
                               _hip.dev_ptr(residual, 'residual') if residual is not None else None,
                               _hip.dev_ptr(out, 'out'), b, sw.c_out, cin, sw.kp, h * w, _hip.stream_ptr())
    return out


def gemm_split_se_route(channels, nblk, c_squeezed, c_out, pixels, aligned=True):
    r = _route(_hip.lib.hs_gemm_split_se_route(channels, nblk, c_squeezed, c_out, pixels, int(bool(aligned))), 'hs_gemm_split_se_route')
    return None if r is None else f'ks{r >> 4}_w{r & 15}'


@_on_operand_device
def gemm_split_se(sw, x, partial, hw, w_reduce, b_reduce, w_expand_t, b_expand, shift=None, act=ACT_NONE, residual=None, out=None,
                  gate_out=None, squeezed_out=None):
    b, cin, h, w = x.shape
    if cin != sw.c_in:
        raise ValueError(f'input has {cin} channels, the weight {sw.c_in}')
    shape = (b, sw.c_out, h, w)
    if out is None:
        out = torch.empty(shape, device=x.device, dtype=torch.float32)
    elif tuple(out.shape) != shape:
        raise ValueError(f'out has shape {tuple(out.shape)}, expected {shape}')
    if residual is not None and tuple(residual.shape) != shape:
        raise ValueError(f'residual has shape {tuple(residual.shape)}, expected {shape}')
    if shift is not None and shift.numel() != sw.c_out:
        raise ValueError(f'shift has {shift.numel()} entries, expected {sw.c_out}')
    if partial.dim() != 2 or partial.shape[0] != b * cin:
        raise ValueError(f'partial has shape {tuple(partial.shape)}, expected ({b * cin}, nblk)')
    csq = w_reduce.shape[0]
    if w_reduce.numel() != csq * cin or b_reduce.numel() != csq:
        raise ValueError(f'w_reduce / b_reduce have {w_reduce.numel()} / {b_reduce.numel()} entries, expected {csq * cin} / {csq}')
    if tuple(w_expand_t.shape) != (csq, cin) or b_expand.numel() != cin:
        raise ValueError(f'w_expand_t has shape {tuple(w_expand_t.shape)} and b_expand {b_expand.numel()} entries, expected {(csq, cin)} and {cin}')
    if gate_out is not None and tuple(gate_out.shape) != (b, cin):
        raise ValueError(f'gate_out has shape {tuple(gate_out.shape)}, expected {(b, cin)}')
    if squeezed_out is not None and tuple(squeezed_out.shape) != (b, csq):
        raise ValueError(f'squeezed_out has shape {tuple(squeezed_out.shape)}, expected {(b, csq)}')
    _hip.run.hs_gemm_split_se_fwd(_hip.dev_ptr(sw.frag, 'w_frag', torch.float16), _hip.dev_ptr(sw.inv, 'w_inv'),
                                  _hip.dev_ptr(partial, 'partial'), partial.shape[1], 1.0 / float(hw),
                                  _hip.dev_ptr(w_reduce, 'w_reduce'), _hip.dev_ptr(b_reduce, 'b_reduce'), csq,
                                  _hip.dev_ptr(w_expand_t, 'w_expand_t'), _hip.dev_ptr(b_expand, 'b_expand'), _hip.dev_ptr(x, 'x'),
                                  _hip.dev_ptr(shift, 'shift') if shift is not None else None, int(act),
                                  _hip.dev_ptr(residual, 'residual') if residual is not None else None,
                                  _hip.dev_ptr(out, 'out'), b, sw.c_out, cin, sw.kp, h * w,
                                  _hip.dev_ptr(gate_out, 'gate_out') if gate_out is not None else None,
                                  _hip.dev_ptr(squeezed_out, 'squeezed_out') if squeezed_out is not None else None, _hip.stream_ptr())
    return out


@_on_operand_device
def gemm_split_conv2x2(sw, x, shift=None, act=ACT_NONE, out=None, pool_partial=None):
    b, cin, h, w = x.shape
    if 4 * cin != sw.c_in:
        raise ValueError(f'input has {cin} channels, the weight {sw.c_in} / 4')
    if h % 2 or w % 4:
        raise ValueError(f'map {h}x{w}: height must be even and width a multiple of 4')
    shape = (b, sw.c_out, h // 2, w // 2)
    if out is None:
        out = torch.empty(shape, device=x.device, dtype=torch.float32)
    elif tuple(out.shape) != shape:
        raise ValueError(f'out has shape {tuple(out.shape)}, expected {shape}')
    if shift is not None and shift.numel() != sw.c_out:
        raise ValueError(f'shift has {shift.numel()} entries, expected {sw.c_out}')
    nblk = -(-(h // 2) * (w // 2) // 16)
    if pool_partial is not None and tuple(pool_partial.shape) != (b, sw.c_out, nblk):
        raise ValueError(f'pool_partial has shape {tuple(pool_partial.shape)}, expected {(b, sw.c_out, nblk)}')
    _hip.run.hs_gemm_split_conv2x2_fwd(_hip.dev_ptr(sw.frag, 'w_frag', torch.float16), _hip.dev_ptr(sw.inv, 'w_inv'),
                                       _hip.dev_ptr(x, 'x'), _hip.dev_ptr(shift, 'shift') if shift is not None else None,
                                       int(act), _hip.dev_ptr(out, 'out'),
                                       _hip.dev_ptr(pool_partial, 'pool_partial') if pool_partial is not None else None,
                                       b, sw.c_out, cin, sw.kp, h // 2, w // 2, _hip.stream_ptr())
    return out


@_on_operand_device
def gemm_split_up2(sw, x, shift=None, act=ACT_NONE, out=None):
    b, cin, h, w = x.shape
    if cin != sw.c_in:
        raise ValueError(f'input has {cin} channels, the weight {sw.c_in}')
    shape = (b, sw.c_out, 2 * h, 2 * w)
    if out is None:
        out = torch.empty(shape, device=x.device, dtype=torch.float32)
    elif tuple(out.shape) != shape:
        raise ValueError(f'out has shape {tuple(out.shape)}, expected {shape}')
    if shift is not None and shift.numel() != sw.c_out:
        raise ValueError(f'shift has {shift.numel()} entries, expected {sw.c_out}')
    _hip.run.hs_gemm_split_up2_fwd(_hip.dev_ptr(sw.frag, 'w_frag', torch.float16), _hip.dev_ptr(sw.inv, 'w_inv'),
                                   _hip.dev_ptr(x, 'x'), _hip.dev_ptr(shift, 'shift') if shift is not None else None,
                                   int(act), _hip.dev_ptr(out, 'out'), b, sw.c_out, cin, sw.kp, h, w, _hip.stream_ptr())
    return out


@_on_operand_device
def pooled_shift(pool_partial, pixels, wb, shift):
    _, c, nblk = pool_partial.shape
    m = shift.numel()
    if pool_partial.shape[0] != 1 or tuple(wb.shape) != (m, c):
        raise ValueError(f'pool_partial {tuple(pool_partial.shape)} / wb {tuple(wb.shape)} / shift {m}: expected (1, C, nblk), (M, C), M')
    out = torch.empty(m, device=shift.device, dtype=torch.float32)
    _hip.run.hs_pooled_shift_fwd(_hip.dev_ptr(pool_partial, 'pool_partial'), nblk, 1.0 / pixels, _hip.dev_ptr(wb, 'wb'),
                                 _hip.dev_ptr(shift, 'shift'), _hip.dev_ptr(out, 'shift_out'), m, c, _hip.stream_ptr())
    return out


@_on_operand_device
def upsample_bilinear(x, size, out=None):
    b, c, hi, wi = x.shape
    ho, wo = size
    if out is not None and tuple(out.shape) == (b, c, ho, wo) and out.dtype == torch.float32 and out.device == x.device and out.is_contiguous():
        y = out
    else:
        y = torch.empty(b, c, ho, wo, device=x.device, dtype=torch.float32)
    _hip.run.hs_upsample_bilinear_fwd(_hip.dev_ptr(x, 'x'), b, c, hi, wi, ho, wo, y.data_ptr(),
                                      _hip.stream_ptr())
    return y


@_on_operand_device
def upsample_argmax(x, size):
    b, c, hi, wi = x.shape
    ho, wo = size
    mask = torch.empty(b, ho, wo, device=x.device, dtype=torch.uint8)
    _hip.run.hs_upsample_argmax_fwd(_hip.dev_ptr(x, 'x'), b, c, hi, wi, ho, wo, mask.data_ptr(), _hip.stream_ptr())
    return mask


_EVAL_DTYPES = {torch.uint8: 0, torch.int64: 1}


def eval_max_classes():
    return int(_hip.lib.hs_eval_max_classes())


def _eval_labels(t, name):
    if not isinstance(t, torch.Tensor) or t.dtype not in _EVAL_DTYPES:
        raise ValueError(f'{name} must be a uint8 or int64 tensor, got {getattr(t, "dtype", type(t))}')
    if not t.is_cuda:
        raise ValueError(f'{name} is on {t.device}: the evaluation kernels run on the GPU (fps.ConfusionMatrix.update counts CPU tensors)')
    return t if t.is_contiguous() else t.contiguous()


def _eval_out(out, shape, device):
    if out is None:
        return torch.zeros(shape, dtype=torch.int64, device=device)
    if not isinstance(out, torch.Tensor) or out.dtype != torch.int64 or tuple(out.shape) != tuple(shape) or out.device != device \
            or not out.is_contiguous():
        raise ValueError(f'out must be a contiguous int64 tensor of shape {tuple(shape)} on {device}, got '
                         f'{getattr(out, "dtype", type(out))} {tuple(getattr(out, "shape", ()))} on {getattr(out, "device", None)}')
    return out


def _eval_classes(num_classes):
    n = int(num_classes)
    if n <= 0:
        raise ValueError(f'num_classes must be positive, got {num_classes}')
    if n > eval_max_classes():
        raise NotImplementedError(f'num_classes = {n}: the evaluation kernels cover up to {eval_max_classes()} classes')
    return n


def _logits_shape(x):
    if not isinstance(x, torch.Tensor) or x.dim() != 4:
        raise ValueError('x must be (B, C, Hi, Wi) logits')
    return x.shape


def _eval_target(target, shape, x):
    target = _eval_labels(target, 'target')
    if tuple(target.shape) != shape:
        raise ValueError(f'target has shape {tuple(target.shape)}, expected {shape}')
    if target.device != x.device:
        raise ValueError(f'target is on {target.device}, the logits on {x.device}')
    return target


def _score_out(num_classes, channels, out, batch, per_image, device, counted=False):
    if counted:
        if channels > int(num_classes):
            raise ValueError(f'{channels} logit channels but num_classes = {num_classes}')
        if int(num_classes) > 256:
            raise ValueError('num_classes > 256: the masks are uint8')
    elif num_classes is None:
        if out is not None:
            raise ValueError('out= needs num_classes: nothing is counted without it')
        if channels > 256:
            raise ValueError('more than 256 logit channels: the masks are uint8')
        return 0, None
    n = _eval_classes(num_classes)
    if channels > n:
        raise ValueError(f'{channels} logit channels but num_classes = {num_classes}')
    return n, _eval_out(out, (batch, n, n) if per_image else (n, n), device)


def _scoring_operands(x, sizes, target, num_classes, out, per_image, counted=False, masks=True, loss=False):
    b, c, hi, wi = _logits_shape(x)
    ho, wo = sizes[-2:]
    target = _eval_target(target, (b, ho, wo), x)
    n, out = _score_out(num_classes, c, out, b, per_image, x.device, counted=counted)
    xp = _hip.dev_ptr(x, 'x')
    loss = torch.empty(b, ho, wo, device=x.device, dtype=torch.float32) if loss else None
    mask = torch.empty(b, ho, wo, device=x.device, dtype=torch.uint8) if masks else None
    head = (xp, b, c, hi, wi, *sizes, target.data_ptr(), _EVAL_DTYPES[target.dtype])
    tail = (n, 1 if per_image else 0, _hip.ptr(out), _hip.ptr(mask), _hip.stream_ptr())
# ... 900 lines not shown
```

### hyperseg_amd/utils/inference.py

```python
import contextlib
import os

import torch
import torch.nn as nn

from ..models._common import Blend, Epilogue, HyperGenBase, Score


class InputNorm:

    LAYOUTS = ('hwc', 'chw')

    def __init__(self, mean=(0.485, 0.456, 0.406), std=(0.229, 0.224, 0.225), layout='hwc'):
        if layout not in self.LAYOUTS:
            raise ValueError(f'layout {layout!r}: expected one of {self.LAYOUTS}')
        self.mean = torch.as_tensor(mean, dtype=torch.float32).flatten().clone()
        self.std = torch.as_tensor(std, dtype=torch.float32).flatten().clone()
        if self.mean.numel() != 3 or self.std.numel() != 3:
            raise ValueError('mean and std must hold one value per channel of a 3-channel frame')
        if bool((self.std == 0).any()):
            raise ValueError('std must be non-zero')
        self.layout = layout
        values = torch.arange(256, dtype=torch.float32)
        self._tables = {torch.device('cpu'): ((values.div(255)[None, :] - self.mean[:, None]) / self.std[:, None]).contiguous()}
# ... 43 lines not shown
        if len(size) != 2 or min(size) < 1:
            raise ValueError(f'size must be (H, W) with both >= 1, got {size}')
        self.size, self.interpolation, self.layout = size, interpolation, layout

    def frame_hw(self, x):
        return (x.shape[1], x.shape[2]) if self.layout == 'hwc' else (x.shape[2], x.shape[3])

    def applies_to(self, x):
        return (isinstance(x, torch.Tensor) and x.dtype == torch.uint8 and x.dim() == 4 and x.shape[3 if self.layout == 'hwc' else 1] == 3
                and tuple(self.frame_hw(x)) != self.size)

    def __call__(self, x, view=None, norm=None, out=None):
        if isinstance(x, torch.Tensor) and x.is_cuda:
            from .. import functional as HF
            return HF.frame_resize(x.contiguous(), self.size, self.interpolation, self.layout, view=view, norm=norm, out=out)
        from . import resample
        got = resample.frame_resize_cpu(x, self.size, self.interpolation, self.layout, view=view, norm=norm)
        if out is not None:
            out.copy_(got)
            got = out
        return got

    def __repr__(self):
        return f'FrameResize(size={self.size}, interpolation={self.interpolation!r}, layout={self.layout!r})'


class Overlay:

    LAYOUTS = InputNorm.LAYOUTS

    def __init__(self, color_map, alpha=0.75, ignore_index=0, layout='hwc'):
        if layout not in self.LAYOUTS:
            raise ValueError(f'layout {layout!r}: expected one of {self.LAYOUTS}')
        cm = torch.as_tensor(color_map)
        if cm.dim() != 2 or cm.shape[1] != 3 or cm.shape[0] < 1:
            raise ValueError(f'color_map must be (n, 3) with n >= 1, got shape {tuple(cm.shape)}')
        if cm.shape[0] > 256:
            raise ValueError(f'color_map has {cm.shape[0]} rows: class indices are uint8, at most 256 colours')
        if cm.is_floating_point() or cm.dtype == torch.bool or cm.is_complex():
            raise ValueError(f'color_map must hold integers in [0, 255], got {cm.dtype}')
        if int(cm.min()) < 0 or int(cm.max()) > 255:
            raise ValueError('color_map must hold integers in [0, 255]')
        alpha = float(alpha)
        if not 0.0 <= alpha <= 1.0:
            raise ValueError(f'alpha must lie in [0, 1], got {alpha}')
        n = cm.shape[0]
        if int(ignore_index) != ignore_index or not -1 <= int(ignore_index) < n:
            raise ValueError(f'ignore_index must be a class of the colour map (0..{n - 1}) or -1 (blend every class), got {ignore_index}')
        self.color_map = cm.to(torch.uint8).cpu().clone()
        self.alpha, self.ignore_index, self.layout = alpha, int(ignore_index), layout
        img = (torch.arange(256, dtype=torch.float32).div(255) - 0.5) / 0.5
        am = 1. - torch.ones((), dtype=torch.float32) * alpha
        self.A1 = img
        self.A = img * am
        self.S = (self.color_map.to(torch.float32).div_(128.).sub_(1.) * (1. - am)).contiguous()
        self._tables = {torch.device('cpu'): torch.cat((self.A, self.A1, self.S.flatten())).contiguous()}

    @property
    def num_colors(self):
        return self.color_map.shape[0]

    def tables(self, device='cpu'):
        device = torch.device(device)
        if device.type == 'cuda' and device.index is None:
            device = torch.device('cuda', torch.cuda.current_device())
        t = self._tables.get(device)
        if t is None:
            t = self._tables[torch.device('cpu')].to(device)
            if device.type == 'cuda' and not torch.cuda.is_current_stream_capturing():
                torch.cuda.current_stream(device).synchronize()
            self._tables[device] = t
        return t

    def frame_size(self, frames):
        if not isinstance(frames, torch.Tensor) or frames.dtype != torch.uint8 or frames.dim() != 4 \
                or frames.shape[3 if self.layout == 'hwc' else 1] != 3:
            want = '(B, H, W, 3)' if self.layout == 'hwc' else '(B, 3, H, W)'
            raise ValueError(f"Overlay(layout='{self.layout}') blends over uint8 frames of shape {want}, got "
                             f'{getattr(frames, "dtype", type(frames))} {tuple(getattr(frames, "shape", ()))}')
        return (frames.shape[0], frames.shape[1], frames.shape[2]) if self.layout == 'hwc' else (frames.shape[0], frames.shape[2], frames.shape[3])

    def check(self, frames, masks):
        size = self.frame_size(frames)
        if not isinstance(masks, torch.Tensor) or masks.dtype != torch.uint8:
            raise ValueError(f'masks must be a uint8 tensor of class indices (segment() returns one; an int64 argmax takes '
                             f'.to(torch.uint8)), got {getattr(masks, "dtype", type(masks))}')
        if tuple(masks.shape) != size:
            raise ValueError(f'masks have shape {tuple(masks.shape)}, the frames are {size} (B, H, W)')
        if masks.device != frames.device:
            raise ValueError(f'masks are on {masks.device}, the frames on {frames.device}')

    def blend(self, frames_u8, masks):
        self.check(frames_u8, masks)
        if frames_u8.is_cuda:
            from .. import functional as HF
            return HF.overlay(masks, frames_u8, self)
        n = self.num_colors
        cls = masks.long()
        blended = ((cls < n) & (cls != self.ignore_index)).unsqueeze(-1)
        v = (frames_u8 if self.layout == 'hwc' else frames_u8.permute(0, 2, 3, 1)).long()
        a = torch.where(blended, self.A[v], self.A1[v])
        s = torch.where(blended, self.S[cls.clamp(max=n - 1)], torch.zeros((), dtype=torch.float32))
        out = (((a + s) * 0.5 + 0.5) * 255.0).round().to(torch.uint8)
        return (out if self.layout == 'hwc' else out.permute(0, 3, 1, 2)).contiguous()

    def __repr__(self):
        return f'Overlay({self.num_colors} colours, alpha={self.alpha}, ignore_index={self.ignore_index}, layout={self.layout!r})'


@torch.no_grad()
def _fold(conv, bn):
    scale = bn.weight / torch.sqrt(bn.running_var + bn.eps)
    shift = bn.bias - bn.running_mean * scale
    conv.weight.mul_(scale.view(-1, 1, 1, 1))
    if conv.bias is not None:
        conv.bias.mul_(scale).add_(shift)
    else:
        conv.bias = nn.Parameter(shift.clone())


def _fold_pairs(module, pairs):
    n = 0
    for conv_name, bn_name in pairs:
        conv, bn = getattr(module, conv_name, None), getattr(module, bn_name, None)
        if isinstance(conv, nn.Conv2d) and isinstance(bn, nn.BatchNorm2d) and not bn.training:
            _fold(conv, bn)
            setattr(module, bn_name, nn.Identity())
            n += 1
    return n


def _fold_sequential(seq):
    n = 0
    mods = list(seq)
    for i in range(len(mods) - 1):
        if isinstance(mods[i], nn.Conv2d) and isinstance(mods[i + 1], nn.BatchNorm2d) and not mods[i + 1].training:
            _fold(mods[i], mods[i + 1])
            seq[i + 1] = nn.Identity()
            n += 1
    return n


def _bn_affine(bn):
    with torch.no_grad():
        scale = bn.weight / torch.sqrt(bn.running_var + bn.eps)
        shift = bn.bias - bn.running_mean * scale
    return scale.detach().clone(), shift.detach().clone()


SPLIT_GEMM_MAX_K = int(os.environ.get('HS_SPLIT_GEMM_MAX_K', '1280'))
STEM_DW = os.environ.get('HS_STEM_DW', '1') != '0'
HS_GEMM_SE = os.environ.get('HS_GEMM_SE', '1') != '0'
GEMM_SE_MAX_CIN = 512
FUSE_EXPAND_MIN_PIXELS = int(os.environ.get('HS_FUSE_EXPAND_MIN_PIXELS', '2048'))
FUSE_EXPAND_MAX_CIN = int(os.environ.get('HS_FUSE_EXPAND_MAX_CIN', '40'))


LEAN_MFMA_MAX_CIN = int(os.environ.get('HS_LEAN_MFMA_MAX_CIN', '16'))
PW_MFMA_MAX_CIN = int(os.environ.get('HS_PW_MFMA_MAX_CIN', '96'))
PW_MFMA_MIN_PIXELS = int(os.environ.get('HS_PW_MFMA_MIN_PIXELS', '8192'))
GEMM_LT_MIN_PIXELS = int(os.environ.get('HS_GEMM_LT_MIN_PIXELS', '16384'))


@contextlib.contextmanager
def gemm_library(pixels, batch=1):
    want = os.environ.get('HS_BLAS') or ('cublaslt' if (pixels >= GEMM_LT_MIN_PIXELS or batch > 1) else 'cublas')
    prev = torch.backends.cuda.preferred_blas_library()
    torch.backends.cuda.preferred_blas_library(want)
    try:
        yield
    finally:
        torch.backends.cuda.preferred_blas_library(prev)


class FusedPointwise(nn.Module):

    def __init__(self, conv, bn, act=0):
        super().__init__()
        assert conv.kernel_size == (1, 1) and conv.stride == (1, 1) and conv.groups == 1 and conv.bias is None
        scale, shift = _bn_affine(bn)
        self.register_buffer('scale', scale, persistent=False)
        self.register_buffer('shift', shift, persistent=False)
        self._conv = [conv]
        self.act = act
        self.split_gemm = False
        self._split = {}

    @property
    def conv(self):
        return self._conv[0]

    def split_weights(self, with_scale, device):
        from .. import functional as HF
        srcs = (self.conv.weight, self.scale) if with_scale else (self.conv.weight,)
        key, ver = (bool(with_scale), device), HF._key(*srcs)
        hit = self._split.get(key)
        if hit is None or hit[0] != ver:
            hit = (ver, HF.gemm_split_weights(self.conv.weight, self.scale if with_scale else None, max_k=SPLIT_GEMM_MAX_K), HF.producer_stream(self.conv.weight.device))
            HF.publish_ready(self.conv.weight.device)
            self._split[key] = hit
        elif hit[1] is not None:
            HF.adopt((hit[1].frag, hit[1].inv), self.conv.weight.device, hit[2])
        return hit[1]

    @torch.no_grad()
    def absorb_input_offset(self, offset):
        w = self.conv.weight.detach().flatten(1).to(offset.device)
        self.shift.add_(self.scale * (w @ offset))

    def uses_mfma(self, x):
        return self.mfma_covers(x.shape[1], x.shape[2] * x.shape[3])

    @staticmethod
    def mfma_covers(channels, pixels):
        return channels <= PW_MFMA_MAX_CIN and pixels >= PW_MFMA_MIN_PIXELS

    def raw(self, x):
        b, cin, h, w = x.shape
        if self.split_gemm:
            sw = self.split_weights(False, x.device)
            if sw is not None:
                from .. import functional as HF
                return HF.gemm_split(sw, x.contiguous())
        with gemm_library(h * w, b):
            if b == 1:
                return torch.mm(self.conv.weight.view(-1, cin), x.view(cin, h * w)).view(1, -1, h, w)
            return torch.bmm(self.conv.weight.view(1, -1, cin).expand(b, -1, -1), x.view(b, cin, h * w)).view(b, -1, h, w)

    def forward(self, x, gate=None, residual=None):
        import torch.nn.functional as F
        from .. import functional as HF
        conv = self.conv
        x = x.contiguous()
        b, cin, h, w = x.shape
        if self.uses_mfma(x):
            return HF.pointwise_conv(x, conv.weight, gate, self.scale, self.shift, self.act, residual)
        if (h * w) % 4 != 0:
            raise NotImplementedError('feature maps with H*W % 4 != 0')
        sw = self.split_weights(True, x.device) if self.split_gemm else None
        if sw is not None:
            return HF.gemm_split(sw, x, gate=gate, shift=self.shift, act=self.act, residual=residual)
        if gate is None:
            y = F.conv2d(x, conv.weight) if b == 1 else self.raw(x)
        else:
            y = F.conv2d(x * gate[:, :, None, None], conv.weight)
        return HF.affine_act_(y, self.scale, self.shift, self.act, residual)


class FusedStem(nn.Module):

    def __init__(self, conv, bn):
        super().__init__()
        assert conv.kernel_size == (3, 3) and conv.stride == (2, 2) and conv.in_channels == 3 and conv.bias is None
        scale, shift = _bn_affine(bn)
        self.register_buffer('scale', scale, persistent=False)
        self.register_buffer('shift', shift, persistent=False)
        self._conv = [conv]
        if conv._pad is not None:
            self.pad_l, self.pad_t = conv._pad[0], conv._pad[2]
            self.pad_w, self.pad_h = conv._pad[0] + conv._pad[1], conv._pad[2] + conv._pad[3]
        else:
            self.pad_t, self.pad_l = conv.padding
            self.pad_h, self.pad_w = 2 * conv.padding[0], 2 * conv.padding[1]
        with torch.no_grad():
            self.register_buffer('w28', nn.functional.pad(conv.weight.detach().flatten(1), (0, 1)).contiguous(), persistent=False)

    def out_size(self, x):
        h, w = x.shape[2:]
        return (h + self.pad_h - 3) // 2 + 1, (w + self.pad_w - 3) // 2 + 1

    def forward(self, x):
        from .. import functional as HF
        x = x.contiguous()
        return HF.stem_conv_bn_swish(x, self._conv[0].weight, self.pad_t, self.pad_l, self.out_size(x), self.scale, self.shift)


class FusedMBConv(nn.Module):

    def __init__(self, blk, in_offset=None, defer_shift=False):
        super().__init__()
        conv = blk._depthwise_conv
        self.expand = FusedPointwise(blk._expand_conv, blk._bn0, act=3) if blk.expand != 1 else None
        self.project = FusedPointwise(blk._project_conv, blk._bn2, act=0)
        scale, shift = _bn_affine(blk._bn1)
        self.register_buffer('scale', scale, persistent=False)
        self.register_buffer('shift', shift, persistent=False)
        self.k, self.stride = conv.kernel_size[0], conv.stride[0]
        if conv._pad is not None:
            self.pad_l, self.pad_t = conv._pad[0], conv._pad[2]
            self.pad_w, self.pad_h = conv._pad[0] + conv._pad[1], conv._pad[2] + conv._pad[3]
        else:
            self.pad_t, self.pad_l = conv.padding
            self.pad_h, self.pad_w = 2 * conv.padding[0], 2 * conv.padding[1]
        self.skip = blk.stride == 1 and blk.in_f == blk.out_f
        self._exp_t = None
        self._red_w = None
        self.se_tail = True
        self._stem = None
        if in_offset is not None:
            assert self.expand is not None, 'a depthwise conv cannot consume an offset tensor (zero padding)'
            self.expand.absorb_input_offset(in_offset)
        with torch.no_grad():
            carried = self.project.shift.clone()
            if self.skip and in_offset is not None:
                carried += in_offset.to(carried.device)
            self.defer_shift = bool(defer_shift)
            self.out_offset = carried.clone() if defer_shift else None
            self.project.shift.copy_(torch.zeros_like(carried) if defer_shift else carried)

    def takes_image(self):
        return self._stem is not None and STEM_DW

    def fuses_expand(self, x, ho, wo):
        return self.expand is not None and x.shape[1] <= FUSE_EXPAND_MAX_CIN and ho * wo >= FUSE_EXPAND_MIN_PIXELS

    def forward(self, inputs, blk):
        from .. import functional as HF
        pre = None
        if self._stem is not None and inputs.shape[1] == 3:
            stem = self._stem[0]
            img = inputs.contiguous()
            pre = HF.stem_dw(img, stem.w28, stem.scale, stem.shift, stem.pad_t, stem.pad_l, stem.out_size(img),
                             blk._depthwise_conv.weight, self.pad_t, self.pad_l, self.scale, self.shift, pool=True) if STEM_DW else None
            if pre is None and isinstance(img, HF.U8Frame):
                img = img.float_image()
            inputs = pre[0] if pre is not None else stem(img)
        x = inputs.contiguous()
        b, _, h, w = x.shape
        ho = (h + self.pad_h - self.k) // self.stride + 1
        wo = (w + self.pad_w - self.k) // self.stride + 1
        lean = True
        red, exp = blk._se_reduce, blk._se_expand
        if self._exp_t is None or self._exp_t.device != x.device:
            self._exp_t = exp.weight.detach().flatten(1).t().contiguous()
        if self._red_w is None or self._red_w.device != x.device:
            self._red_w = red.weight.detach().flatten(1)
        proj = self.project
        cmid = blk._depthwise_conv.weight.shape[0]
        lean_gemm = lean and (cmid > LEAN_MFMA_MAX_CIN if self.defer_shift else not proj.mfma_covers(cmid, ho * wo))
        folds = lean_gemm and not (proj.split_gemm and proj.split_weights(True, x.device) is not None)
        se = (self._red_w, red.bias, self._exp_t, exp.bias) if self.se_tail and not folds else None
        if pre is not None:
            out = (pre[0], pre[1], False) if se is not None else pre
        elif self.fuses_expand(x, ho, wo):
            out = HF.mbconv_expand_dw(x, self.expand.conv.weight, self.expand.scale, self.expand.shift,
                                      blk._depthwise_conv.weight, self.stride, self.pad_t, self.pad_l, (ho, wo),
                                      self.scale, self.shift, pool=True, se=se)
        else:
            in_scale = in_shift = None
            if self.expand is not None:
                if lean and not self.expand.uses_mfma(x):
                    in_scale, in_shift = self.expand.scale, self.expand.shift
                    x = self.expand.raw(x)
                else:
                    x = self.expand(x)
            out = HF.depthwise_conv_bn_act(x, blk._depthwise_conv.weight, self.stride, self.pad_t, self.pad_l,
                                           (ho, wo), self.scale, self.shift, act=3, pool=True,
                                           in_scale=in_scale, in_shift=in_shift, se=se)
        y, pooled, gated = out if se is not None else (out[0], out[1], False)

        def se_gate(**fold):
            if gated and not fold:
                return pooled
            return HF.se_gate(pooled, b, ho * wo, red.weight, red.bias, self._exp_t, exp.bias, **fold)
        skip = inputs.contiguous() if self.skip else None
        if lean_gemm:
            sw = proj.split_weights(True, y.device) if proj.split_gemm else None
            if sw is not None:
                if (HS_GEMM_SE and y.is_cuda and not gated and cmid <= GEMM_SE_MAX_CIN and
                        HF.gemm_split_se_route(cmid, pooled.shape[1], self._red_w.shape[0], sw.c_out, ho * wo,
                                               aligned=(pooled.data_ptr() | red.weight.data_ptr()) % 16 == 0) is not None):
                    se_ops = (pooled, ho * wo, red.weight, red.bias, self._exp_t, exp.bias)
                    if self.defer_shift:
                        if skip is None:
                            return HF.gemm_split_se(sw, y, *se_ops)
                        return HF.gemm_split_se(sw, y, *se_ops, residual=skip, out=skip)
                    return HF.gemm_split_se(sw, y, *se_ops, shift=proj.shift, residual=skip)
                gate = se_gate()
                if self.defer_shift:
                    if skip is None:
                        return HF.gemm_split(sw, y, gate=gate)
                    return HF.gemm_split(sw, y, gate=gate, residual=skip, out=skip)
                return HF.gemm_split(sw, y, gate=gate, shift=proj.shift, residual=skip)
            wp = se_gate(w_proj=proj.conv.weight, out_scale=proj.scale)
            cmid = y.shape[1]
            with gemm_library(ho * wo, b):
                if b == 1:
                    w2d, y2d = wp.view(-1, cmid), y.view(cmid, ho * wo)
                    if self.defer_shift:
                        if skip is None:
                            return torch.mm(w2d, y2d).view(1, -1, ho, wo)
                        skip.view(-1, ho * wo).addmm_(w2d, y2d)
                        return skip
                    out = torch.mm(w2d, y2d).view(1, -1, ho, wo)
                else:
                    w3d, y3d = wp.view(b, -1, cmid), y.view(b, cmid, ho * wo)
                    if self.defer_shift:
                        if skip is None:
                            return torch.bmm(w3d, y3d).view(b, -1, ho, wo)
                        skip.view(b, -1, ho * wo).baddbmm_(w3d, y3d)
                        return skip
                    out = torch.bmm(w3d, y3d).view(b, -1, ho, wo)
            return HF.affine_act_(out, None, proj.shift, 0, skip)
        return proj(y, gate=se_gate(), residual=skip)


CTX_DOWN_SPLIT = os.environ.get('HS_CTX_DOWN_SPLIT', '1') != '0'


class FusedContextHead(nn.Module):

    def __init__(self, wm):
        super().__init__()
        self._wm = [wm]
        blocks = [wm.in_conv] + list(wm.down_blocks) + list(wm.up_blocks)
        for i, blk in enumerate(blocks):
            assert isinstance(blk[0], nn.Conv2d) and isinstance(blk[1], nn.BatchNorm2d) and isinstance(blk[2], nn.ReLU)
            assert blk[0].bias is None
            scale, shift = _bn_affine(blk[1])
            self.register_buffer(f'scale{i}', scale, persistent=False)
            self.register_buffer(f'shift{i}', shift, persistent=False)
        self.n_down = n = len(wm.down_blocks)
        with torch.no_grad():
            up = wm.up_blocks[n - 1]
            half = up[0].out_channels
            wb = up[0].weight.detach().flatten(1)[:, half:]
            self.register_buffer('wb_scaled', getattr(self, f'scale{2 * n}')[:, None] * wb, persistent=False)

        self.split_gemm = False
        self._split = {}

    def _affine(self, i):
        return getattr(self, f'scale{i}'), getattr(self, f'shift{i}')

    def _split_weights(self, name, weight, scale, max_k=1280):
        from .. import functional as HF
        key = HF._key(weight, scale)
        hit = self._split.get(name)
        if hit is None or hit[0] != key:
            hit = (key, HF.gemm_split_weights(weight, scale, max_k=max_k), HF.producer_stream(weight.device))
            HF.publish_ready(weight.device)
            self._split[name] = hit
        elif hit[1] is not None:
            HF.adopt((hit[1].frag, hit[1].inv), weight.device, hit[2])
        return hit[1]

    def forward(self, x):
        with gemm_library(x.shape[2] * x.shape[3]):
            return self._forward(x)

    def _forward(self, x):
        from .. import functional as HF
        import torch.nn.functional as F
        wm = self._wm[0]
        _, cin, h, w = x.shape
        half = cin // 2
        n = self.n_down
        signal = torch.empty(1, cin, h, w, device=x.device, dtype=torch.float32)
        left = signal[:, :half]
        sw_in = self._split_weights('in', wm.in_conv[0].weight.view(half, cin), self.scale0) if self.split_gemm and (h * w) % 4 == 0 else None
        if sw_in is not None:
            HF.gemm_split(sw_in, x.contiguous(), shift=self.shift0, act=HF.ACT_RELU, out=left)
        else:
            torch.mm(wm.in_conv[0].weight.view(half, cin), x.view(cin, h * w), out=left.view(half, h * w))
            HF.affine_act_(left, *self._affine(0), HF.ACT_RELU)
        feat = [left]
        pool = None
        for i, down in enumerate(wm.down_blocks):
            src = feat[-1]
            sw_dn = None
            if self.split_gemm and CTX_DOWN_SPLIT and src.shape[2] % 2 == 0 and src.shape[3] % 4 == 0 and src.is_contiguous() and src.data_ptr() % 16 == 0:
                sw_dn = self._split_weights(f'down{i}', down[0].weight, getattr(self, f'scale{1 + i}'), max_k=2560)
            if sw_dn is not None:
                ho, wo = src.shape[2] // 2, src.shape[3] // 2
                if i == n - 1 and (ho, wo) != (1, 1):
                    pool = torch.empty(1, half, -(-ho * wo // 16), device=x.device, dtype=torch.float32)
                feat.append(HF.gemm_split_conv2x2(sw_dn, src, shift=getattr(self, f'shift{1 + i}'), act=HF.ACT_RELU, pool_partial=pool))
            else:
                t = F.conv2d(src, down[0].weight, stride=2)
                feat.append(HF.affine_act_(t, *self._affine(1 + i), HF.ACT_RELU))
        t = feat[-1]
        pooled_const = t.shape[-2:] != (1, 1)
        for level in range(n - 1, -1, -1):
            up = wm.up_blocks[level]
            scale, shift = self._affine(1 + n + level)
            wgt = up[0].weight.view(half, cin)
            skip = feat.pop()
            sh, sw = skip.shape[-2:]
            if pooled_const:
                if pool is not None:
                    shift = HF.pooled_shift(pool, t.shape[2] * t.shape[3], self.wb_scaled, shift)
                else:
                    shift = torch.addmv(shift, self.wb_scaled, t.mean((2, 3)).view(half))
                sw_up = self._split_weights(f'up{level}', wgt[:, :half], scale) if self.split_gemm and (sh * sw) % 4 == 0 else None
                if sw_up is not None and level == 0:
                    HF.gemm_split_up2(sw_up, skip.contiguous(), shift=shift, act=HF.ACT_RELU, out=signal[:, half:])
                    return signal
                if sw_up is not None:
                    y = HF.gemm_split(sw_up, skip.contiguous(), shift=shift, act=HF.ACT_RELU)
                else:
                    y = HF.affine_act_(torch.mm(wgt[:, :half], skip.view(half, sh * sw)).view(1, half, sh, sw), scale, shift, HF.ACT_RELU)
                pooled_const = False
            else:
                y = torch.mm(wgt, torch.cat((skip, t), dim=1).view(cin, sh * sw)).view(1, half, sh, sw)
                y = HF.affine_act_(y, scale, shift, HF.ACT_RELU)
            if level > 0:
                t = wm.upsample(y)
            else:
                signal[:, half:].view(half, sh, 2, sw, 2).copy_(y.view(half, sh, 1, sw, 1).expand(half, sh, 2, sw, 2))
        return signal


def _fuse_backbone(bb):
    blocks = list(bb._blocks)
    offset, tap = None, 0
    bb._fused_fc = nn.ModuleDict()
    for idx, blk in enumerate(blocks):
        conv = blk._depthwise_conv
        ok = conv.kernel_size[0] in (3, 5) and conv.stride[0] in (1, 2) and isinstance(blk._bn1, nn.BatchNorm2d)
        tapped = bb._res_feat_mask[idx]
        fc = getattr(bb, f'_feat_fc_{tap}', None) if (tapped and bb.out_feat_scale is not None) else None
        if ok:
            nxt = blocks[idx + 1] if idx + 1 < len(blocks) else None
            nxt_ok = nxt is None or (nxt.expand != 1 and nxt._depthwise_conv.kernel_size[0] in (3, 5)
                                     and isinstance(nxt._bn1, nn.BatchNorm2d))
            defer = nxt_ok and (not tapped or isinstance(fc, nn.Sequential))
            blk._fused_dw = FusedMBConv(blk, in_offset=offset, defer_shift=defer)
            offset = blk._fused_dw.out_offset
        else:
            assert offset is None
# ... 351 lines not shown
```

### include/hyperseg_hip.h

```cpp
#ifndef HYPERSEG_HIP_H
#define HYPERSEG_HIP_H

#include <stdint.h>

#ifdef __cplusplus
extern "C" {
#endif

#define HS_ABI_VERSION 1

typedef enum {
    HS_OK = 0,
    HS_ERR_BAD_ARG = -1,
    HS_ERR_NOT_DIVISIBLE = -2,
    HS_ERR_UNSUPPORTED = -3,
    HS_ERR_LDS = -4
} hs_status;

typedef enum { HS_ACT_NONE = 0, HS_ACT_RELU = 1, HS_ACT_RELU6 = 2, HS_ACT_SWISH = 3 } hs_act;
typedef enum { HS_PAD_ZEROS = 0, HS_PAD_REFLECT = 1, HS_PAD_REPLICATE = 2, HS_PAD_CIRCULAR = 3 } hs_pad_mode;
typedef enum { HS_PREV_NONE = 0, HS_PREV_SAME = 1, HS_PREV_BILINEAR = 2 } hs_prev_mode;

typedef struct {
    const float* skip;
// ... 240 lines not shown
int hs_stem_dw_fwd(const float* x, int32_t batch, int32_t H, int32_t W, const float* w_stem28, int32_t c_mid,
                   const float* scale0, const float* shift0, int32_t stem_pad_t, int32_t stem_pad_l, int32_t Hs, int32_t Ws,
                   const float* w_dw, int32_t k, int32_t pad_t, int32_t pad_l, const float* scale1, const float* shift1,
                   float* y, float* pool_partial, void* stream);
#define HS_LAYOUT_HWC 0
#define HS_LAYOUT_CHW 1
int hs_image_ingest_fwd(const uint8_t* x, int32_t layout, int32_t batch, int32_t channels, int32_t H, int32_t W, const float* table,
                        float* y, void* stream);
int hs_stem_dw_u8_fwd(const uint8_t* x, int32_t layout, const float* table, int32_t batch, int32_t H, int32_t W,
                      const float* w_stem28, int32_t c_mid, const float* scale0, const float* shift0, int32_t stem_pad_t,
                      int32_t stem_pad_l, int32_t Hs, int32_t Ws, const float* w_dw, int32_t k, int32_t pad_t, int32_t pad_l,
                      const float* scale1, const float* shift1, float* y, float* pool_partial, void* stream);
int hs_overlay_fwd(const uint8_t* masks, const uint8_t* frames, int32_t layout, int32_t batch, int32_t H, int32_t W,
                   const float* tables, int32_t num_colors, int32_t ignore_index, uint8_t* overlay, void* stream);
int hs_upsample_overlay_fwd(const float* x, int32_t batch, int32_t channels, int32_t Hi, int32_t Wi, int32_t Ho, int32_t Wo,
                            const uint8_t* frames, int32_t layout, const float* tables, int32_t num_colors, int32_t ignore_index,
                            uint8_t* mask, uint8_t* overlay, void* stream);
int hs_upsample2_overlay_fwd(const float* x, int32_t batch, int32_t channels, int32_t Hi, int32_t Wi, int32_t Hm, int32_t Wm, int32_t Ho,
                             int32_t Wo, const uint8_t* frames, int32_t layout, const float* tables, int32_t num_colors,
                             int32_t ignore_index, uint8_t* mask, uint8_t* overlay, void* stream);
typedef enum { HS_CONF_F32 = 0, HS_CONF_U8 = 1 } hs_conf_dtype;
int hs_confidence_fwd(const float* logits, int32_t batch, int32_t channels, int32_t H, int32_t W, int32_t conf_dtype, float threshold,
                      int32_t fill, uint8_t* mask, void* conf, void* stream);
int hs_upsample_confidence_fwd(const float* x, int32_t batch, int32_t channels, int32_t Hi, int32_t Wi, int32_t Ho, int32_t Wo,
                               int32_t conf_dtype, float threshold, int32_t fill, uint8_t* mask, void* conf, void* stream);
int hs_upsample2_confidence_fwd(const float* x, int32_t batch, int32_t channels, int32_t Hi, int32_t Wi, int32_t Hm, int32_t Wm, int32_t Ho,
                                int32_t Wo, int32_t conf_dtype, float threshold, int32_t fill, uint8_t* mask, void* conf, void* stream);
int hs_frame_resize_fwd(const uint8_t* x, int32_t layout, int32_t batch, int32_t Hi, int32_t Wi,
                        const int32_t* y_bounds, const int32_t* y_kk, int32_t y_ksize, int32_t Hr,
                        const int32_t* x_bounds, const int32_t* x_kk, int32_t x_ksize, int32_t Wr,
                        int32_t Ho, int32_t Wo, int32_t oy, int32_t ox, int32_t hflip, uint32_t fill_rgb,
                        const float* norm_table, void* y, void* stream);
int hs_label_resize_fwd(const void* x, int32_t in_dtype, int32_t batch, int32_t Hi, int32_t Wi,
                        const int32_t* y_index, int32_t Hr, const int32_t* x_index, int32_t Wr,
                        int32_t Ho, int32_t Wo, int32_t oy, int32_t ox, int32_t hflip, int32_t fill,
                        void* y, int32_t out_dtype, void* stream);
#define HS_RESIZE_BILINEAR 0
#define HS_RESIZE_BICUBIC 1
#define HS_RESIZE_STATUS_HR 1
#define HS_RESIZE_STATUS_WR 2
#define HS_RESIZE_STATUS_Y_TAPS 4
#define HS_RESIZE_STATUS_X_TAPS 8
#define HS_RESIZE_STATUS_SIZE 16
int hs_resize_tables_fwd(const int32_t* params, int32_t batch, int32_t Hi, int32_t Wi, int32_t Ho, int32_t Wo, int32_t filter,
                         int32_t ks_max, int32_t* bounds, int32_t* kk, int32_t* nearest, int32_t* status, void* stream);
int hs_frame_resize_batch_fwd(const uint8_t* x, int32_t layout, int32_t batch, int32_t Hi, int32_t Wi, const int32_t* params,
                              const int32_t* bounds, const int32_t* kk, const int32_t* status, int32_t ks_max,
                              int32_t Ho, int32_t Wo, uint32_t fill_rgb, const float* norm_table, void* y, void* stream);
int hs_label_resize_batch_fwd(const void* x, int32_t in_dtype, int32_t batch, int32_t Hi, int32_t Wi, const int32_t* params,
                              const int32_t* nearest, const int32_t* status, int32_t Ho, int32_t Wo, int32_t fill,
                              void* y, int32_t out_dtype, void* stream);
#define HS_CODEC_NONE 0
#define HS_CODEC_TABLE 1
#define HS_CODEC_COLORS 2
int hs_label_encode_fwd(const void* x, int32_t in_kind, int32_t batch, int32_t H, int32_t W, const int32_t* codec_words,
                        int32_t codec_kind, int32_t n, int32_t unmatched, void* y, int32_t out_dtype, void* stream);
int hs_label_resize_coded_fwd(const void* x, int32_t in_dtype, int32_t batch, int32_t Hi, int32_t Wi,
                              const int32_t* y_index, int32_t Hr, const int32_t* x_index, int32_t Wr,
                              int32_t Ho, int32_t Wo, int32_t oy, int32_t ox, int32_t hflip, int32_t fill,
                              const int32_t* codec_words, int32_t codec_kind, int32_t n, int32_t unmatched,
                              void* y, int32_t out_dtype, void* stream);
int hs_label_resize_batch_coded_fwd(const void* x, int32_t in_dtype, int32_t batch, int32_t Hi, int32_t Wi, const int32_t* params,
                                    const int32_t* nearest, const int32_t* status, int32_t Ho, int32_t Wo, int32_t fill,
                                    const int32_t* codec_words, int32_t codec_kind, int32_t n, int32_t unmatched,
                                    void* y, int32_t out_dtype, void* stream);
#define HS_JITTER_TABLE_WORDS 8
int hs_color_jitter_fwd(const uint8_t* x, int32_t layout, int32_t batch, int32_t H, int32_t W, const int32_t* table,
                        uint64_t* sums, const float* norm_table, void* y, void* stream);
#define HS_BLUR_TABLE_WORDS 4
#define HS_BLUR_MAX_RADIUS 15
#define HS_BLUR_MAX_DIM 32768
#define HS_BLUR_STATUS_RADIUS 1
int hs_gaussian_blur_fwd(const uint8_t* x, int32_t layout, int32_t batch, int32_t H, int32_t W, const int32_t* table,
                         uint8_t* tmp, const float* norm_table, void* y, int32_t* status, void* stream);
int hs_frame_rotate_fwd(const uint8_t* x, int32_t layout, int32_t batch, int32_t H, int32_t W, const double* matrices,
                        int32_t Ho, int32_t Wo, uint32_t fill_rgb, uint32_t pad_fill_rgb, const float* norm_table,
                        void* y, void* stream);
int hs_label_rotate_fwd(const void* x, int32_t in_dtype, int32_t batch, int32_t H, int32_t W, const int32_t* fixed,
                        int32_t Ho, int32_t Wo, int32_t fill, int32_t pad_fill, void* y, int32_t out_dtype, void* stream);
#define HS_RAGGED_PARAM_WORDS 8
#define HS_RESIZE_STATUS_EXTENT 32
#define HS_RESIZE_STATUS_CANVAS 64
int hs_resize_tables_ragged_fwd(const int32_t* params, int32_t batch, int32_t Hm, int32_t Wm, int32_t Hc, int32_t Wc, int32_t filter,
                                int32_t ks_max, int32_t* bounds, int32_t* kk, int32_t* nearest, int32_t* status, void* stream);
int hs_color_jitter_ragged_fwd(const uint8_t* x, int32_t layout, int32_t batch, int32_t Hm, int32_t Wm, const int32_t* params,
                               const int32_t* table, uint64_t* sums, uint8_t* y, void* stream);
int hs_frame_resize_ragged_fwd(const uint8_t* x, int32_t layout, int32_t batch, int32_t Hm, int32_t Wm, const int32_t* params,
                               const int32_t* bounds, const int32_t* kk, const int32_t* status, int32_t ks_max,
                               int32_t Hc, int32_t Wc, uint8_t* y, void* stream);
int hs_label_resize_ragged_fwd(const void* x, int32_t in_dtype, int32_t batch, int32_t Hm, int32_t Wm, const int32_t* params,
                               const int32_t* nearest, const int32_t* status, int32_t Hc, int32_t Wc, uint8_t* y, void* stream);
int hs_frame_rotate_ragged_fwd(const uint8_t* x, int32_t layout, int32_t batch, int32_t Hc, int32_t Wc, const int32_t* params,
                               const int32_t* status, const double* matrices, int32_t Ho, int32_t Wo, uint32_t fill_rgb,
                               uint32_t pad_fill_rgb, const float* norm_table, void* y, void* stream);
int hs_label_rotate_ragged_fwd(const uint8_t* x, int32_t batch, int32_t Hc, int32_t Wc, const int32_t* params, const int32_t* status,
                               const int32_t* fixed, int32_t Ho, int32_t Wo, int32_t fill, int32_t pad_fill, void* y, int32_t out_dtype,
                               void* stream);
int hs_mbconv_expand_dw_fwd(const float* x, int32_t batch, int32_t c_in, int32_t H, int32_t W,
                            const float* w_expand, int32_t c_mid, const float* scale0, const float* shift0,
                            const float* w_dw, int32_t k, int32_t stride, int32_t pad_t, int32_t pad_l,
                            int32_t Ho, int32_t Wo, const float* scale1, const float* shift1, float* y,
                            float* pool_partial, void* stream);
int64_t hs_mbconv_se_workgroups(int32_t batch, int32_t c_mid, int32_t k, int32_t stride, int32_t Ho, int32_t Wo);
int hs_mbconv_expand_dw_se_fwd(const float* x, int32_t batch, int32_t c_in, int32_t H, int32_t W,
                               const float* w_expand, int32_t c_mid, const float* scale0, const float* shift0,
                               const float* w_dw, int32_t k, int32_t stride, int32_t pad_t, int32_t pad_l,
                               int32_t Ho, int32_t Wo, const float* scale1, const float* shift1, float* y,
                               const hs_se_tail* se, void* stream);

int hs_pointwise_conv_fwd(const float* x, int32_t batch, int32_t c_in, int32_t pixels, const float* w, int32_t c_out,
                          const float* gate, const float* scale, const float* shift, int32_t act, const float* residual,
                          float* y, void* stream);

int hs_affine_act_fwd(const float* x, int32_t batch, int32_t channels, int32_t pixels, const float* scale,
                      const float* shift, int32_t act, const float* residual, float* y, void* stream);

#define HS_DW_FORM_GENERIC 0
#define HS_DW_FORM_VECTOR 1
#define HS_DW_FORM_TILED 2
#define HS_DW_ROUTE(form, k, stride, pl) (((form) << 8) | ((k) << 4) | ((stride) << 2) | (pl))
int hs_depthwise_route(int32_t batch, int32_t channels, int32_t H, int32_t W, int32_t k, int32_t stride, int32_t pad_l,
                       int32_t Ho, int32_t Wo, int32_t x_aligned16, int32_t prologue);
#define HS_STEM_ROUTE_GENERIC 0
#define HS_STEM_ROUTE_VECTOR_PL0 1
#define HS_STEM_ROUTE_VECTOR_PL1 2
int hs_stem_route(int32_t W, int32_t pad_l, int32_t x_aligned16);
#define HS_MB_FORM_FULL 0
#define HS_MB_FORM_LEAN 1
#define HS_MB_FORM_STEM 2
#define HS_MB_ROUTE(form, k, stride) (((form) << 8) | ((k) << 4) | (stride))
int hs_mbconv_route(int32_t batch, int32_t c_in, int32_t H, int32_t W, int32_t c_mid, int32_t k, int32_t stride,
                    int32_t Ho, int32_t Wo, int32_t aligned16, int32_t with_se_tail);
int hs_stem_dw_route(int32_t H, int32_t W, int32_t c_mid, int32_t stem_pad_t, int32_t stem_pad_l, int32_t Hs, int32_t Ws,
                     int32_t k, int32_t aligned16);
#define HS_SE_ROUTE_FUSED 0
#define HS_SE_ROUTE_EARLY 1
#define HS_SE_ROUTE_FUSED_WIDE 2
#define HS_SE_ROUTE_TWO_LAUNCH 3
int hs_se_gate_route(int32_t channels, int32_t nblk, int32_t c_squeezed, int32_t with_w_proj, int32_t aligned16);
#define HS_PW_ROUTE(nb, nt, vec) (((nb) << 8) | ((nt) << 4) | (vec))
int hs_pointwise_route(int32_t batch, int32_t c_in, int32_t c_out, int32_t pixels, int32_t aligned16);

int hs_gemm_split_kp(int32_t c_in);
int hs_gemm_split_fwd(const void* w_frag, const float* w_inv, const float* gate, const float* x, const float* shift,
                      int32_t act, const float* residual, float* y, int32_t batch, int32_t c_out, int32_t c_in, int32_t kp,
                      int32_t pixels, void* stream);
#define HS_GSE_ROUTE(ks, nwv) (((ks) << 4) | (nwv))
int hs_gemm_split_se_fwd(const void* w_frag, const float* w_inv, const float* partial, int32_t nblk, float inv_hw,
                         const float* w_reduce, const float* b_reduce, int32_t c_squeezed, const float* w_expand_t,
                         const float* b_expand, const float* x, const float* shift, int32_t act, const float* residual,
                         float* y, int32_t batch, int32_t c_out, int32_t c_in, int32_t kp, int32_t pixels,
                         float* gate_out, float* squeezed_out, void* stream);
int hs_gemm_split_se_route(int32_t channels, int32_t nblk, int32_t c_squeezed, int32_t c_out, int32_t pixels, int32_t aligned16);
int hs_gemm_split_conv2x2_fwd(const void* w_frag, const float* w_inv, const float* x, const float* shift, int32_t act, float* y,
                              float* pool_partial, int32_t batch, int32_t c_out, int32_t c_in, int32_t kp, int32_t Ho,
                              int32_t Wo, void* stream);
int hs_gemm_split_up2_fwd(const void* w_frag, const float* w_inv, const float* x, const float* shift, int32_t act, float* y,
                          int32_t batch, int32_t c_out, int32_t c_in, int32_t kp, int32_t Ho, int32_t Wo, void* stream);
int hs_pooled_shift_fwd(const float* partial, int32_t nblk, float inv_pixels, const float* wb, const float* shift,
                        float* shift_out, int32_t rows, int32_t channels, void* stream);

int hs_halo_tiles_fwd(int32_t dtype, const void* x, int32_t batch, int32_t channels, int32_t H, int32_t W, int32_t fh, int32_t fw,
                      void* tiled, int32_t patch_major, void* stream);
int hs_halo_tiles_bwd(int32_t dtype, const void* dtiled, int32_t batch, int32_t channels, int32_t H, int32_t W, int32_t fh, int32_t fw,
                      void* dx, int32_t patch_major, void* stream);
int hs_tile_interior_fwd(int32_t dtype, const void* tiled, int32_t batch, int32_t channels, int32_t H, int32_t W, int32_t fh,
                         int32_t fw, void* y, void* stream);
int hs_tile_interior_bwd(int32_t dtype, const void* dy, int32_t batch, int32_t channels, int32_t H, int32_t W, int32_t fh, int32_t fw,
                         void* dtiled, void* stream);
int hs_dw_tiles_fwd(int32_t dtype, const void* tiled, const float* bank, int64_t ld, int32_t batch, int32_t channels, int32_t H, int32_t W,
                    int32_t fh, int32_t fw, void* y, int32_t patch_major, void* stream);
int hs_dw_tiles_bwd_in(int32_t dtype, const void* dy, const float* bank, int64_t ld, int32_t batch, int32_t channels, int32_t H, int32_t W,
                       int32_t fh, int32_t fw, void* dtiled, int32_t patch_major, void* stream);
int hs_dw_tiles_bwd_w(int32_t dtype, const void* tiled, const void* dy, int32_t batch, int32_t channels, int32_t H, int32_t W, int32_t fh,
                      int32_t fw, float* dbank, int64_t ld, int32_t patch_major, void* stream);
int64_t hs_bootstrap_mean_workspace(void);
int hs_bootstrap_mean_of_batch_fwd(const float* values, int32_t images, int32_t n, int32_t k, float thresh, void* workspace,
                                   float* out8, float* mean_out, void* stream);
int hs_bootstrap_mean_of_batch_bwd(const float* values, int32_t images, int32_t n, const float* state8, const float* grad_mean,
                                   float* grad_values, void* stream);
int64_t hs_adam_blocks(const int64_t* numel, int32_t n);
int hs_adam_step(float* const* params, const float* const* grads, float* const* exp_avg, float* const* exp_avg_sq, const int64_t* numel,
                 int32_t n, const float* lr_device, float lr, double beta1, double beta2, float eps, float weight_decay, int32_t decoupled,
                 int32_t maximize, float* steps, void* stream);
int hs_adam_step_amp(float* const* params, float* const* grads, float* const* exp_avg, float* const* exp_avg_sq, const int64_t* numel,
                     int32_t n, const float* lr_device, float lr, double beta1, double beta2, float eps, float weight_decay, int32_t decoupled,
                     int32_t maximize, float* steps, const float* grad_scale, const float* found_inf, void* stream);
int hs_bootstrap_mean_fwd(const float* values, int32_t n, int32_t k, float thresh, void* workspace, float* out5, void* stream);
int hs_bootstrap_mean_bwd(const float* values, int32_t n, const float* state5, const float* grad_out, float* grad_values, void* stream);
int hs_bootstrap_mean_batched_fwd(const float* values, int32_t images, int32_t n, int32_t k, float thresh, void* workspace, float* out8,
                                  void* stream);
int hs_bootstrap_mean_batched_bwd(const float* values, int32_t images, int32_t n, const float* state8, const float* grad_out,
                                  float* grad_values, void* stream);

int hs_bank_unpack_fwd(const float* bank, int64_t ld, int32_t batch, int32_t hp_total, int32_t fh, int32_t fw, int32_t ch_offset,
                       int32_t rows, float* w, void* stream);

int hs_upsample_bilinear_bwd(const float* dy, int64_t dy_batch_stride, int32_t batch, int32_t channels, int32_t Hi, int32_t Wi,
                             int32_t Ho, int32_t Wo, float* dx, void* stream);
int hs_upsample_bilinear_typed_bwd(int32_t dtype, const void* dy, int64_t dy_batch_stride, int32_t batch, int32_t channels, int32_t Hi,
                                   int32_t Wi, int32_t Ho, int32_t Wo, void* dx, void* stream);

int64_t hs_bn_train_workspace(int32_t channels);
int hs_bn_train_stats_fwd(int32_t dtype, const void* x, int32_t batch, int32_t channels, int64_t pixels, void* workspace, void* stream);
int hs_dw_tiles_bn_fwd(int32_t dtype, const void* tiled, const float* bn_partial, const float* gamma, const float* beta,
                       float* running_mean, float* running_var, float momentum, float eps, int32_t act, float* save_mean,
                       float* save_invstd, int64_t* num_batches_tracked, const float* bank, int64_t ld, int32_t batch,
                       int32_t channels, int32_t H, int32_t W, int32_t fh, int32_t fw, void* y, int32_t patch_major, void* stream);
int hs_dw_tiles_bn_bwd_w(int32_t dtype, const void* tiled, const void* dy, const float* gamma, const float* beta, const float* save_mean,
                         const float* save_invstd, int32_t act, int32_t batch, int32_t channels, int32_t H, int32_t W, int32_t fh,
                         int32_t fw, float* dbank, int64_t ld, int32_t patch_major, void* stream);
int hs_patch_conv_bn_fwd(int32_t dtype, const void* x, const float* bn_partial, const float* gamma, const float* beta,
                         float* running_mean, float* running_var, float momentum, float eps, int32_t act, float* save_mean,
                         float* save_invstd, int64_t* num_batches_tracked, const float* bank, int64_t ld, int32_t batch,
                         int32_t c_in, int32_t H, int32_t W, int32_t fh, int32_t fw, int32_t c_out, void* y, void* stream);
int hs_patch_conv_bn_bwd_w(int32_t dtype, const void* x, const void* dy, const float* gamma, const float* beta, const float* save_mean,
                           const float* save_invstd, int32_t act, int32_t batch, int32_t c_in, int32_t H, int32_t W, int32_t fh,
                           int32_t fw, int32_t c_out, float* dbank, int64_t ld, void* stream);
int hs_bn_act_train_fwd(int32_t dtype, const void* x, int32_t batch, int32_t channels, int64_t pixels, const float* gamma,
                        const float* beta, float* running_mean, float* running_var, float momentum, float eps, int32_t act,
                        float* save_mean, float* save_invstd, void* workspace, void* y, int64_t* num_batches_tracked, void* stream);
int hs_bn_act_train_bwd(int32_t dtype, const void* x, const void* dy, int32_t batch, int32_t channels, int64_t pixels,
                        const float* gamma, const float* beta, const float* save_mean, const float* save_invstd, float eps, int32_t act,
                        void* workspace, void* dx, float* dgamma, float* dbeta, void* stream);
int64_t hs_dw_tiles_bn_bwd_in_partials(int32_t batch, int32_t H, int32_t W, int32_t fh, int32_t fw);
int hs_dw_tiles_bn_bwd_in(int32_t dtype, const void* dy, const float* bank, int64_t ld, const void* tiled, const float* gamma, const float* beta,
                          const float* save_mean, const float* save_invstd, int32_t act, int32_t batch, int32_t channels, int32_t H, int32_t W,
                          int32_t fh, int32_t fw, void* dtiled, float* partial, int32_t patch_major, void* stream);
int hs_bn_act_train_bwd_apply(int32_t dtype, const void* x, const void* dy, int32_t batch, int32_t channels, int64_t pixels, const float* gamma,
                              const float* beta, const float* save_mean, const float* save_invstd, int32_t act, const float* partial,
                              int64_t n_partials, void* dx, float* dgamma, float* dbeta, void* stream);

typedef struct hs_s2w_train_layer {
    int32_t signal_index, signal_channels, groups;
    const float* w;
    int32_t wc, rows;
    float* bank;
    int64_t ld;
    const float* dbank;
    float* dw;
    float* ds;
} hs_s2w_train_layer;
int hs_s2w_train_fwd(const float* signal, int32_t batch, int32_t c_signal, int32_t fh, int32_t fw,
                     const hs_s2w_train_layer* layers, int32_t n_layers, void* stream);
int64_t hs_s2w_train_workspace(int32_t batch, int32_t fh, int32_t fw, const hs_s2w_train_layer* layers, int32_t n_layers);
int hs_s2w_train_bwd(const float* signal, int32_t batch, int32_t c_signal, int32_t fh, int32_t fw,
                     const hs_s2w_train_layer* layers, int32_t n_layers, float* dsignal, void* workspace, int64_t workspace_bytes,
                     void* stream);

int hs_cross_entropy_fwd(const float* logits, const int64_t* target, int32_t batch, int32_t classes, int64_t pixels,
                         int64_t ignore_index, float* loss, void* stream);
int hs_cross_entropy_bwd(const float* logits, const int64_t* target, int32_t batch, int32_t classes, int64_t pixels,
                         int64_t ignore_index, const float* grad_loss, float* grad_logits, void* stream);
int hs_cross_entropy_typed_fwd(int32_t dtype, const void* logits, const int64_t* target, int32_t batch, int32_t classes, int64_t pixels,
                               int64_t ignore_index, float* loss, void* stream);
int hs_cross_entropy_typed_bwd(int32_t dtype, const void* logits, const int64_t* target, int32_t batch, int32_t classes, int64_t pixels,
                               int64_t ignore_index, const float* grad_loss, void* grad_logits, void* stream);
int hs_bootstrapped_ce_fwd(int32_t dtype, const void* logits, const int64_t* target, int32_t batch, int32_t classes, int64_t pixels,
                           int64_t ignore_index, int32_t k, float thresh, void* workspace, float* loss, float* out8, float* mean_out, void* stream);
int hs_bootstrapped_ce_bwd(int32_t dtype, const void* logits, const int64_t* target, int32_t batch, int32_t classes, int64_t pixels,
                           int64_t ignore_index, const float* loss, const float* state8, const float* grad_mean, void* grad_logits, void* stream);
int hs_cross_entropy_weighted_fwd(int32_t dtype, const void* logits, const int64_t* target, const float* weight, int32_t batch, int32_t classes,
                                  int64_t pixels, int64_t ignore_index, float* loss, void* stream);
int hs_cross_entropy_weighted_bwd(int32_t dtype, const void* logits, const int64_t* target, const float* weight, int32_t batch, int32_t classes,
                                  int64_t pixels, int64_t ignore_index, const float* grad_loss, void* grad_logits, void* stream);
int hs_bootstrapped_ce_weighted_fwd(int32_t dtype, const void* logits, const int64_t* target, const float* weight, int32_t batch,
                                    int32_t classes, int64_t pixels, int64_t ignore_index, int32_t k, float thresh, void* workspace, float* loss,
                                    float* out8, float* mean_out, void* stream);
int hs_bootstrapped_ce_weighted_bwd(int32_t dtype, const void* logits, const int64_t* target, const float* weight, int32_t batch,
                                    int32_t classes, int64_t pixels, int64_t ignore_index, const float* loss, const float* state8,
                                    const float* grad_mean, void* grad_logits, void* stream);

int hs_stage_input_fwd(const hs_stage_input* in, float* y, void* stream);
int hs_stage_input_typed_fwd(const hs_stage_input* in, int32_t prev_dtype, int32_t out_dtype, void* y, void* stream);

#ifdef __cplusplus
}
#endif
#endif
```

Before: 1369.

## Add squeeze-then-fused-excite GEMM path and restructure SE gate expand compute

Adds a kernel variant that takes a precomputed SE squeeze vector and folds the excite (expand plus sigmoid) into the project GEMM prologue. It also adds a standalone squeeze launch. This is meant to replace the two-launch SE path for wider channel counts. The existing fused SE-gate kernel now computes the expand as quad-split partial chains with cross-lane reduction. The new excite route is gated by a max-channel constant set to zero, so it is disabled by default.

Measured after the change: 1376 (median of 6 runs). About the same (+0.5%).

```diff
diff --git a/hyperseg_amd/_hip.py b/hyperseg_amd/_hip.py
--- a/hyperseg_amd/_hip.py
+++ b/hyperseg_amd/_hip.py
@@ -209,6 +209,9 @@
     'hs_gemm_split_fwd': ([vp, vp, vp, vp, vp, i32, vp, vp, i32, i32, i32, i32, i32, vp], STATUS),
     'hs_gemm_split_se_fwd': ([vp, vp, vp, i32, C.c_float, vp, vp, i32, vp, vp, vp, vp, i32, vp, vp, i32, i32, i32, i32, i32, vp, vp, vp], STATUS),
     'hs_gemm_split_se_route': ([i32] * 6, C.c_int),
+    'hs_gemm_split_excite_fwd': ([vp, vp, vp, i32, vp, vp, vp, vp, i32, vp, vp, i32, i32, i32, i32, i32, vp, vp], STATUS),
+    'hs_gemm_split_excite_route': ([i32] * 5, C.c_int),
+    'hs_se_squeeze_fwd': ([vp, i32, i32, i32, C.c_float, vp, vp, i32, vp, vp], STATUS),
     'hs_gemm_split_conv2x2_fwd': ([vp, vp, vp, vp, i32, vp, vp, i32, i32, i32, i32, i32, i32, vp], STATUS),
     'hs_gemm_split_up2_fwd': ([vp, vp, vp, vp, i32, vp, i32, i32, i32, i32, i32, i32, vp], STATUS),
     'hs_depthwise_route': ([i32] * 11, C.c_int),
diff --git a/hyperseg_amd/csrc/hs_encoder.hip b/hyperseg_amd/csrc/hs_encoder.hip
--- a/hyperseg_amd/csrc/hs_encoder.hip
+++ b/hyperseg_amd/csrc/hs_encoder.hip
@@ -639,6 +639,15 @@
     return launch_status();
 }
 
+extern "C" int hs_se_squeeze_fwd(const float* partial, int32_t batch, int32_t channels, int32_t nblk, float inv_hw, const float* w_reduce,
+                                 const float* b_reduce, int32_t c_squeezed, float* squeezed, void* stream) {
+    if (!partial || !w_reduce || !b_reduce || !squeezed || batch <= 0 || channels <= 0 || nblk <= 0 || c_squeezed <= 0) return HS_ERR_BAD_ARG;
+    if (batch > 65535 || c_squeezed > 65535) return HS_ERR_UNSUPPORTED;
+    hipLaunchKernelGGL(se_squeeze_kernel, dim3(c_squeezed, batch), dim3(256), 0, (hipStream_t)stream, partial, nblk, inv_hw, w_reduce,
+                       b_reduce, channels, c_squeezed, squeezed);
+    return launch_status();
+}
+
 namespace hs {
 
 using f32x4 = __attribute__((ext_vector_type(4))) float;
diff --git a/hyperseg_amd/csrc/hs_gemm_split.hip b/hyperseg_amd/csrc/hs_gemm_split.hip
--- a/hyperseg_amd/csrc/hs_gemm_split.hip
+++ b/hyperseg_amd/csrc/hs_gemm_split.hip
@@ -31,8 +31,18 @@
     float* gate_out; float* squeezed_out;
     float inv_hw; int nblk, Csq;
 };
-template <bool SEG> struct GemmSeOperand {};
-template <> struct GemmSeOperand<true> : GemmSeArgs {};
+struct GemmExciteArgs {
+    const float* __restrict__ z;
+    const float* __restrict__ w2t; const float* __restrict__ b2;
+    float* gate_out;
+    int Csq;
+};
+enum GsSe : int { GS_SE_NONE = 0, GS_SE_GATE = 1, GS_SE_EXCITE = 2 };
+template <int SEG> struct GemmSeOperand {};
+template <> struct GemmSeOperand<GS_SE_GATE> : GemmSeArgs {};
+template <> struct GemmSeOperand<GS_SE_EXCITE> : GemmExciteArgs {};
+constexpr int GSX_MAX_K = 1280, GSX_MAX_CSQ = 64;
+constexpr int GSX_ZS = 0, GSX_GATE = GSX_ZS + GSX_MAX_CSQ, GSX_LDS_FLOATS = GSX_GATE + GSX_MAX_K;
 
 #ifndef HS_GS_NARROW_MAX_WG
 #define HS_GS_NARROW_MAX_WG 128
@@ -42,10 +52,11 @@
 #define HS_GS_TALL_MIN_WG 257
 #endif
 
-template <int KS, int NWV, bool FAST, int NS, int MT, int NCH, bool PATCH, bool SEG = false>
+template <int KS, int NWV, bool FAST, int NS, int MT, int NCH, bool PATCH, int SEG = GS_SE_NONE>
 __global__ __launch_bounds__(64 * NWV)
 void gemm_split_kernel(GemmSplitArgs a, GemmSeOperand<SEG> se) {
-    static_assert(!SEG || (FAST && !PATCH && NCH == 1 && (NWV == 8 ? KS <= 3 : KS == 1)), "SEG: the project convolutions' forms only");
+    static_assert(SEG != GS_SE_GATE || (FAST && !PATCH && NCH == 1 && (NWV == 8 ? KS <= 3 : KS == 1)), "SEG: the project convolutions' forms only");
+    static_assert(SEG != GS_SE_EXCITE || (FAST && !PATCH && NCH == 1 && NWV == 8 && KS <= 5), "EXCITE: the project convolutions' forms only");
     extern __shared__ __attribute__((aligned(16))) float gs_red[];
     constexpr int nthr = 64 * NWV, nwv = NWV;
     constexpr int NP = 16 * NS, NR = 16 * MT, NE = NR * NP;
@@ -82,7 +93,8 @@
                         xv[c][1][s][2 * q] = v[2]; xv[c][1][s][2 * q + 1] = v[3];
                     }
                 }
-    } else {
+    }
+    auto load_x = [&]() {
 #pragma unroll
         for (int c = 0; c < NCH; ++c)
 #pragma unroll
@@ -100,7 +112,8 @@
                         xv[c][0][s][j] = xb[(size_t)kc * a.N + ncol0]; xv[c][1][s][j] = xb[(size_t)kc * a.N + ncol1];
                     }
                 }
-    }
+    };
+    if constexpr (!PATCH && SEG != GS_SE_EXCITE) load_x();
     constexpr int NG = PATCH ? 1 : NCH;
     float gv[NG][KS][8];
     if constexpr (!PATCH) {
@@ -109,7 +122,7 @@
 #pragma unroll
             for (int s = 0; s < KS; ++s) {
                 const int k0 = ((wave * NCH + c) * KS + s) * 32 + 8 * kg;
-                if constexpr (SEG) {
+                if constexpr (SEG != GS_SE_NONE) {
                 } else if constexpr (FAST) {
                     const float* gp = gb ? gb + min(k0, a.K - 8) : a.w_inv;
                     const gs_f32x4 g0 = *reinterpret_cast<const gs_f32x4*>(gp), g1 = *reinterpret_cast<const gs_f32x4*>(gp + 4);
@@ -131,7 +144,7 @@
             al[q & 1][s] = *reinterpret_cast<const half8*>(blk + 512);
         }
     };
-    load_a(0);
+    if constexpr (SEG != GS_SE_EXCITE) load_a(0);
     constexpr int TE = (NE + nthr - 1) / nthr;
     float wi[TE], sh[TE], yo[TE];
     auto load_tail = [&]() {
@@ -145,34 +158,68 @@
         }
     };
     constexpr bool LATE_TAIL = KS * NCH >= 3;
-    if constexpr (!LATE_TAIL) load_tail();
+    if constexpr (!LATE_TAIL && SEG != GS_SE_EXCITE) load_tail();
     constexpr int SE_PV = SEP_MAX_UNITS / nthr, SE_RW = SEP_MAX_CSQ / NWV, SE_W1U = NWV == 8 ? (KS < 3 ? KS : 3) : 1;
-    constexpr int SE_CI = NWV == 8 && KS >= 3 ? 2 : 1;
-    float4 se_pv[SE_PV], se_w1v[SE_RW][SE_W1U];
-    float se_b1v[SE_RW], se_w2q[SE_CI][4][8], se_b2v[SE_CI];
-    if constexpr (SEG) {
+    constexpr int SE_CI = SEG == GS_SE_EXCITE ? (KS + 1) / 2 : (NWV == 8 && KS >= 3 ? 2 : 1);
+    constexpr int SE_ROWS = SEG == GS_SE_EXCITE ? 4 : 8;
+    float4 se_pv[SE_PV], se_w1v[SE_RW][SE_W1U], se_w2v[SE_CI][SE_ROWS];
+    float se_b1v[SE_RW], se_b2v[SE_CI], se_zv = 0.0f;
+    if constexpr (SEG == GS_SE_GATE) {
         se_load_units<nthr, SE_PV>(se.partial + (size_t)b * a.K * se.nblk, se.nblk, a.K, tid, se_pv);
         se_load_reduce<NWV, SE_RW, SE_W1U>(se.w1, se.b1, a.K, se.Csq, wave, lane, se_w1v, se_b1v);
-#pragma unroll
-        for (int ci = 0; ci < SE_CI; ++ci) se_load_expand(se.w2t, se.b2, a.K, se.Csq, min(tid + nthr * ci, a.K - 1), se_w2q[ci], se_b2v[ci]);
+        se_load_expand_quads<nthr, SE_CI, SE_ROWS>(se.w2t, a.K, se.Csq, tid, 0, se_w2v);
+        se_load_expand_bias<nthr, SE_CI>(se.b2, a.K, tid, se_b2v);
+    }
+    if constexpr (SEG == GS_SE_EXCITE) {
+        se_zv = se.z[(size_t)b * se.Csq + min(tid, se.Csq - 1)];
+        se_load_expand_quads<nthr, SE_CI, SE_ROWS>(se.w2t, a.K, se.Csq, tid, 0, se_w2v);
+        se_load_expand_bias<nthr, SE_CI>(se.b2, a.K, tid, se_b2v);
     }
     __builtin_amdgcn_sched_barrier(0);
-    if constexpr (SEG) {
+    if constexpr (SEG == GS_SE_EXCITE) {
+        float* zs = gs_red + GSX_ZS; float* gate_s = gs_red + GSX_GATE;
+        if (tid < se.Csq) zs[tid] = se_zv;
+        __syncthreads();
+        float4 se_q[SE_CI];
+#pragma unroll
+        for (int n = 0; n < SE_CI; ++n) se_q[n] = make_float4(0.0f, 0.0f, 0.0f, 0.0f);
+        se_quarter_chains<nthr, SE_CI, SE_ROWS>(se_w2v, zs, a.K, se.Csq, tid, 0, se_q);
+#pragma unroll
+        for (int u0 = SE_ROWS; u0 < GSX_MAX_CSQ / 4; u0 += SE_ROWS) {
+            __builtin_amdgcn_sched_barrier(0);
+            se_load_expand_quads<nthr, SE_CI, SE_ROWS>(se.w2t, a.K, se.Csq, tid, u0, se_w2v);
+            __builtin_amdgcn_sched_barrier(0);
+            se_quarter_chains<nthr, SE_CI, SE_ROWS>(se_w2v, zs, a.K, se.Csq, tid, u0, se_q);
+        }
+        __builtin_amdgcn_sched_barrier(0);
+        load_x();
+        load_a(0);
+        if constexpr (!LATE_TAIL) load_tail();
+        __builtin_amdgcn_sched_barrier(0);
+        const bool first = blockIdx.x == 0 && blockIdx.y == 0;
+        se_quad_gates<nthr, SE_CI>(se_q, se_b2v, a.K, tid, gate_s, first && se.gate_out ? se.gate_out + (size_t)b * a.K : nullptr);
+        __syncthreads();
+#pragma unroll
+        for (int s = 0; s < KS; ++s) {
+            const float* gp = gate_s + min((wave * KS + s) * 32 + 8 * kg, a.K - 8);
+            const gs_f32x4 g0 = *reinterpret_cast<const gs_f32x4*>(gp), g1 = *reinterpret_cast<const gs_f32x4*>(gp + 4);
+#pragma unroll
+            for (int j = 0; j < 4; ++j) { gv[0][s][j] = g0[j]; gv[0][s][4 + j] = g1[j]; }
+        }
+        __syncthreads();
+    }
+    if constexpr (SEG == GS_SE_GATE) {
         float* mean_c = gs_red + SEP_MEAN; float* zs = gs_red + SEP_ZS; float* gate_s = gs_red + SEP_GATE;
         se_channel_means<nthr, SE_PV>(se_pv, se.nblk, a.K, se.inv_hw, tid, gs_red + SEP_PART, mean_c);
         se_squeeze_rows<NWV, SE_RW, SE_W1U>(se_w1v, se_b1v, mean_c, a.K, se.Csq, wave, lane, zs);
         __syncthreads();
         const bool first = blockIdx.x == 0 && blockIdx.y == 0;
         if (first && se.squeezed_out && tid < se.Csq) se.squeezed_out[(size_t)b * se.Csq + tid] = zs[tid];
-#pragma unroll
-        for (int ci = 0; ci < SE_CI; ++ci) {
-            const int ch = tid + nthr * ci;
-            const float g = se_channel_gate(se_w2q[ci], se_b2v[ci], zs, se.Csq);
-            if (ch < a.K) {
-                gate_s[ch] = g;
-                if (first && se.gate_out) se.gate_out[(size_t)b * a.K + ch] = g;
-            }
-        }
+        float4 se_q[SE_CI];
+#pragma unroll
+        for (int n = 0; n < SE_CI; ++n) se_q[n] = make_float4(0.0f, 0.0f, 0.0f, 0.0f);
+        se_quarter_chains<nthr, SE_CI, SE_ROWS>(se_w2v, zs, a.K, se.Csq, tid, 0, se_q);
+        se_quad_gates<nthr, SE_CI>(se_q, se_b2v, a.K, tid, gate_s, first && se.gate_out ? se.gate_out + (size_t)b * a.K : nullptr);
         __syncthreads();
 #pragma unroll
         for (int s = 0; s < KS; ++s) {
@@ -199,7 +246,7 @@
                 for (int j = 0; j < 8; ++j) {
                     const float mk = (FAST || PATCH ? k0 : k0 + j) < a.K ? 1.0f : 0.0f;
                     float g = mk;
-                    if constexpr (!PATCH) g = SEG || gb ? gv[c][s][j] * mk : mk;
+                    if constexpr (!PATCH) g = SEG != GS_SE_NONE || gb ? gv[c][s][j] * mk : mk;
                     xv[c][t][s][j] *= g;
                     mx = max(mx, __float_as_uint(xv[c][t][s][j]) & 0x7fffffffu);
                 }
@@ -394,15 +441,15 @@
     GemmSplitArgs a{(const _Float16*)w_frag, w_inv, gate, x, shift, residual, y, c_out, c_in, kp / 32, pixels, act, 0, nullptr, up2_wo};
     hipStream_t s = (hipStream_t)stream;
 #define HS_GS_(KSV, NWV, F) do { \
-        if (narrow) hipLaunchKernelGGL((gemm_split_kernel<KSV, NWV, F, 1, 2, 1, false>), grid, dim3(64 * NWV), lds, s, a, GemmSeOperand<false>{}); \
-        else if (tall) hipLaunchKernelGGL((gemm_split_kernel<KSV, NWV, F, 2, 4, 1, false>), grid, dim3(64 * NWV), lds, s, a, GemmSeOperand<false>{}); \
-        else hipLaunchKernelGGL((gemm_split_kernel<KSV, NWV, F, 2, 2, 1, false>), grid, dim3(64 * NWV), lds, s, a, GemmSeOperand<false>{}); } while (0)
+        if (narrow) hipLaunchKernelGGL((gemm_split_kernel<KSV, NWV, F, 1, 2, 1, false>), grid, dim3(64 * NWV), lds, s, a, GemmSeOperand<GS_SE_NONE>{}); \
+        else if (tall) hipLaunchKernelGGL((gemm_split_kernel<KSV, NWV, F, 2, 4, 1, false>), grid, dim3(64 * NWV), lds, s, a, GemmSeOperand<GS_SE_NONE>{}); \
+        else hipLaunchKernelGGL((gemm_split_kernel<KSV, NWV, F, 2, 2, 1, false>), grid, dim3(64 * NWV), lds, s, a, GemmSeOperand<GS_SE_NONE>{}); } while (0)
 #define HS_GS(KSV, NWV) do { if (fast) HS_GS_(KSV, NWV, true); else HS_GS_(KSV, NWV, false); } while (0)
     if (nch == 2) {
         if (!fast || up2_wo > 0) return HS_ERR_UNSUPPORTED;
         grid.x = (pixels + 15) / 16; grid.y = ((c_out + 15) / 16 + 1) / 2;
         const size_t lds2 = (size_t)8 * 512 * sizeof(float);
-#define HS_GS2(KSV) hipLaunchKernelGGL((gemm_split_kernel<KSV, 8, true, 1, 2, 2, false>), grid, dim3(512), lds2, s, a, GemmSeOperand<false>{})
+#define HS_GS2(KSV) hipLaunchKernelGGL((gemm_split_kernel<KSV, 8, true, 1, 2, 2, false>), grid, dim3(512), lds2, s, a, GemmSeOperand<GS_SE_NONE>{})
         switch (ks) { case 3: HS_GS2(3); break; case 4: HS_GS2(4); break; case 5: HS_GS2(5); break; default: return HS_ERR_UNSUPPORTED; }
 #undef HS_GS2
         return launch_status();
@@ -445,25 +492,72 @@
     if (!partial || !w_reduce || !b_reduce || !w_expand_t || !b_expand || nblk <= 0 || c_squeezed <= 0) return HS_ERR_BAD_ARG;
     if (act < 0 || act > 3) return HS_ERR_BAD_ARG;
     GemmSplitPolicy pol;
-    const bool aligned16 = (((size_t)partial | (size_t)w_reduce) & 15) == 0;
+    const bool aligned16 = (((size_t)partial | (size_t)w_reduce | (size_t)w_expand_t) & 15) == 0;
     const int route = gemm_split_se_route(c_in, nblk, c_squeezed, c_out, pixels, aligned16, batch, pol);
     if (route < 0) return route;
     if (kp != pol.nwv * pol.ks * 32) return HS_ERR_BAD_ARG;
     GemmSplitArgs a{(const _Float16*)w_frag, w_inv, nullptr, x, shift, residual, y, c_out, c_in, kp / 32, pixels, act, 0, nullptr, 0};
-    GemmSeOperand<true> se{{partial, w_reduce, b_reduce, w_expand_t, b_expand, gate_out, squeezed_out, inv_hw, nblk, c_squeezed}};
+    GemmSeOperand<GS_SE_GATE> se{{partial, w_reduce, b_reduce, w_expand_t, b_expand, gate_out, squeezed_out, inv_hw, nblk, c_squeezed}};
     const size_t se_lds = (size_t)SEP_LDS_FLOATS * sizeof(float);
     const size_t lds = pol.lds > se_lds ? pol.lds : se_lds;
     hipStream_t s = (hipStream_t)stream;
 #define HS_GSE(KSV, NWV) do { \
-        if (pol.narrow) hipLaunchKernelGGL((gemm_split_kernel<KSV, NWV, true, 1, 2, 1, false, true>), pol.grid, dim3(64 * NWV), lds, s, a, se); \
-        else if (pol.tall) hipLaunchKernelGGL((gemm_split_kernel<KSV, NWV, true, 2, 4, 1, false, true>), pol.grid, dim3(64 * NWV), lds, s, a, se); \
-        else hipLaunchKernelGGL((gemm_split_kernel<KSV, NWV, true, 2, 2, 1, false, true>), pol.grid, dim3(64 * NWV), lds, s, a, se); } while (0)
+        if (pol.narrow) hipLaunchKernelGGL((gemm_split_kernel<KSV, NWV, true, 1, 2, 1, false, GS_SE_GATE>), pol.grid, dim3(64 * NWV), lds, s, a, se); \
+        else if (pol.tall) hipLaunchKernelGGL((gemm_split_kernel<KSV, NWV, true, 2, 4, 1, false, GS_SE_GATE>), pol.grid, dim3(64 * NWV), lds, s, a, se); \
+        else hipLaunchKernelGGL((gemm_split_kernel<KSV, NWV, true, 2, 2, 1, false, GS_SE_GATE>), pol.grid, dim3(64 * NWV), lds, s, a, se); } while (0)
     switch (pol.ks) {
         case 1: if (pol.nwv == 2) HS_GSE(1, 2); else if (pol.nwv == 4) HS_GSE(1, 4); else HS_GSE(1, 8); break;
         case 2: HS_GSE(2, 8); break;
         default: HS_GSE(3, 8); break;
     }
 #undef HS_GSE
+    return launch_status();
+}
+
+static int gemm_split_excite_route(int channels, int c_squeezed, int c_out, int pixels, bool aligned16, int batch, GemmSplitPolicy& pol) {
+    if (channels <= 0 || c_squeezed <= 0 || c_out <= 0 || pixels <= 0 || batch <= 0) return HS_ERR_BAD_ARG;
+    const int kp = hs_gemm_split_kp(channels);
+    if (kp < 0) return HS_ERR_UNSUPPORTED;
+    const int pst = gemm_split_policy(batch, c_out, channels, kp, pixels, pol);
+    if (pst != HS_OK) return pst;
+    if (!aligned16 || !pol.fast || pol.nch != 1 || pol.nwv != 8 || pol.ks > 5) return HS_ERR_UNSUPPORTED;
+    if (channels > GSX_MAX_K || c_squeezed > GSX_MAX_CSQ || (channels & 3) != 0) return HS_ERR_UNSUPPORTED;
+    return HS_GSE_ROUTE(pol.ks, pol.nwv);
+}
+
+extern "C" int hs_gemm_split_excite_route(int32_t channels, int32_t c_squeezed, int32_t c_out, int32_t pixels, int32_t aligned16) {
+    GemmSplitPolicy pol;
+    return gemm_split_excite_route(channels, c_squeezed, c_out, pixels, aligned16 != 0, 1, pol);
+}
+
+extern "C" int hs_gemm_split_excite_fwd(const void* w_frag, const float* w_inv, const float* squeezed, int32_t c_squeezed,
+                                        const float* w_expand_t, const float* b_expand, const float* x, const float* shift, int32_t act,
+                                        const float* residual, float* y, int32_t batch, int32_t c_out, int32_t c_in, int32_t kp,
+                                        int32_t pixels, float* gate_out, void* stream) {
+    if (!w_frag || !w_inv || !x || !y || batch <= 0 || c_out <= 0 || c_in <= 0 || pixels <= 0) return HS_ERR_BAD_ARG;
+    if (!squeezed || !w_expand_t || !b_expand || c_squeezed <= 0) return HS_ERR_BAD_ARG;
+    if (act < 0 || act > 3) return HS_ERR_BAD_ARG;
+    GemmSplitPolicy pol;
+    const int route = gemm_split_excite_route(c_in, c_squeezed, c_out, pixels, (((size_t)w_expand_t) & 15) == 0, batch, pol);
+    if (route < 0) return route;
+    if (kp != pol.nwv * pol.ks * 32) return HS_ERR_BAD_ARG;
+    GemmSplitArgs a{(const _Float16*)w_frag, w_inv, nullptr, x, shift, residual, y, c_out, c_in, kp / 32, pixels, act, 0, nullptr, 0};
+    GemmSeOperand<GS_SE_EXCITE> se{{squeezed, w_expand_t, b_expand, gate_out, c_squeezed}};
+    const size_t se_lds = (size_t)GSX_LDS_FLOATS * sizeof(float);
+    const size_t lds = pol.lds > se_lds ? pol.lds : se_lds;
+    hipStream_t s = (hipStream_t)stream;
+#define HS_GSX(KSV) do { \
+        if (pol.narrow) hipLaunchKernelGGL((gemm_split_kernel<KSV, 8, true, 1, 2, 1, false, GS_SE_EXCITE>), pol.grid, dim3(512), lds, s, a, se); \
+        else if (pol.tall) hipLaunchKernelGGL((gemm_split_kernel<KSV, 8, true, 2, 4, 1, false, GS_SE_EXCITE>), pol.grid, dim3(512), lds, s, a, se); \
+        else hipLaunchKernelGGL((gemm_split_kernel<KSV, 8, true, 2, 2, 1, false, GS_SE_EXCITE>), pol.grid, dim3(512), lds, s, a, se); } while (0)
+    switch (pol.ks) {
+        case 1: HS_GSX(1); break;
+        case 2: HS_GSX(2); break;
+        case 3: HS_GSX(3); break;
+        case 4: HS_GSX(4); break;
+        default: HS_GSX(5); break;
+    }
+#undef HS_GSX
     return launch_status();
 }
 
@@ -504,7 +598,7 @@
     dim3 grid((pixels + 15) / 16, ((c_out + 15) / 16 + 1) / 2, batch);
     const size_t lds = (size_t)8 * 512 * sizeof(float);
     hipStream_t s = (hipStream_t)stream;
-#define HS_GP(KSV, NCHV) hipLaunchKernelGGL((gemm_split_kernel<KSV, 8, true, 1, 2, NCHV, true>), grid, dim3(512), lds, s, a, GemmSeOperand<false>{})
+#define HS_GP(KSV, NCHV) hipLaunchKernelGGL((gemm_split_kernel<KSV, 8, true, 1, 2, NCHV, true>), grid, dim3(512), lds, s, a, GemmSeOperand<GS_SE_NONE>{})
     switch (ks * 2 + nch - 1) {
         case 2: HS_GP(1, 1); break;
         case 4: HS_GP(2, 1); break;
diff --git a/hyperseg_amd/csrc/hs_se_gate_phases.h b/hyperseg_amd/csrc/hs_se_gate_phases.h
--- a/hyperseg_amd/csrc/hs_se_gate_phases.h
+++ b/hyperseg_amd/csrc/hs_se_gate_phases.h
@@ -85,29 +85,67 @@
     }
 }
 
-__device__ __forceinline__ void se_load_expand(const float* __restrict__ w2t, const float* __restrict__ b2, int C, int Csq, int c,
-                                               float (&w2q)[4][8], float& b2v) {
-    const int jq = (Csq + 3) >> 2;
+template <int NTHR, int NJ, int ROWS>
+__device__ __forceinline__ void se_load_expand_quads(const float* __restrict__ w2t, int C, int Csq, int tid, int u0, float4 (&w2v)[NJ][ROWS]) {
+    const int jq = (Csq + 3) >> 2, c4 = C >> 2;
 #pragma unroll
-    for (int i = 0; i < 4; ++i)
+    for (int n = 0; n < NJ; ++n) {
+        const int g = tid + NTHR * n, cq = min(g >> 2, c4 - 1), i = g & 3;
 #pragma unroll
-        for (int u = 0; u < 8; ++u) w2q[i][u] = w2t[(size_t)min(i * jq + u, Csq - 1) * C + c];
-    b2v = b2[c];
+        for (int u = 0; u < ROWS; ++u) {
+            w2v[n][u] = make_float4(0.0f, 0.0f, 0.0f, 0.0f);
+            if (NTHR * n < C && u0 + u < jq)
+                w2v[n][u] = reinterpret_cast<const float4*>(w2t + (size_t)min(i * jq + u0 + u, Csq - 1) * C)[cq];
+        }
+    }
 }
 
-__device__ __forceinline__ float se_channel_gate(const float (&w2q)[4][8], float b2v, const float* zs, int Csq) {
-    const int jq = (Csq + 3) >> 2;
-    float q[4];
+template <int NTHR, int NJ>
+__device__ __forceinline__ void se_load_expand_bias(const float* __restrict__ b2, int C, int tid, float (&b2v)[NJ]) {
 #pragma unroll
-    for (int i = 0; i < 4; ++i) {
-        const int j0 = i * jq, j1 = min(j0 + jq, Csq);
-        float acc = 0.0f;
+    for (int n = 0; n < NJ; ++n) b2v[n] = b2[min(tid + NTHR * n, C - 1)];
+}
+
+template <int NTHR, int NJ, int ROWS>
+__device__ __forceinline__ void se_quarter_chains(const float4 (&w2v)[NJ][ROWS], const float* zs, int C, int Csq, int tid, int u0, float4 (&q)[NJ]) {
+    const int jq = (Csq + 3) >> 2, j0 = (tid & 3) * jq, j1 = min(j0 + jq, Csq);
 #pragma unroll
-        for (int u = 0; u < 8; ++u)
-            if (j0 + u < j1) acc = fmaf(w2q[i][u], zs[min(j0 + u, SEP_MAX_CSQ - 1)], acc);
-        q[i] = acc;
+    for (int u = 0; u < ROWS; ++u) {
+        const bool live = j0 + u0 + u < j1;
+        const float z = zs[min(j0 + u0 + u, Csq - 1)];
+#pragma unroll
+        for (int n = 0; n < NJ; ++n) {
+            if (NTHR * n < C && live) {
+                q[n].x = fmaf(w2v[n][u].x, z, q[n].x); q[n].y = fmaf(w2v[n][u].y, z, q[n].y);
+                q[n].z = fmaf(w2v[n][u].z, z, q[n].z); q[n].w = fmaf(w2v[n][u].w, z, q[n].w);
+            }
+        }
     }
-    return sigmoidf_fast(((q[0] + q[1]) + (q[2] + q[3])) + b2v);
+}
+
+template <int NTHR, int NJ>
+__device__ __forceinline__ void se_quad_gates(const float4 (&q)[NJ], const float (&b2v)[NJ], int C, int tid, float* gate_s, float* gate_out) {
+    const int i = tid & 3;
+    auto xor1 = [](float v) { return __int_as_float(__builtin_amdgcn_update_dpp(0, __float_as_int(v), 0xB1, 0xf, 0xf, false)); };
+    auto xor2 = [](float v) { return __int_as_float(__builtin_amdgcn_update_dpp(0, __float_as_int(v), 0x4E, 0xf, 0xf, false)); };
+    auto total = [&](float v) {
+        const float o = xor1(v), pair = (i & 1) ? o + v : v + o;
+        const float p = xor2(pair);
+        return (i & 2) ? p + pair : pair + p;
+    };
+#pragma unroll
+    for (int n = 0; n < NJ; ++n) {
+        if (NTHR * n < C) {
+            const float tx = total(q[n].x), ty = total(q[n].y), tz = total(q[n].z), tw = total(q[n].w);
+            const float t = i == 0 ? tx : (i == 1 ? ty : (i == 2 ? tz : tw));
+            const float g = sigmoidf_fast(t + b2v[n]);
+            const int ch = tid + NTHR * n;
+            if (ch < C) {
+                gate_s[ch] = g;
+                if (gate_out) gate_out[ch] = g;
+            }
+        }
+    }
 }
 
 }
diff --git a/hyperseg_amd/functional.py b/hyperseg_amd/functional.py
--- a/hyperseg_amd/functional.py
+++ b/hyperseg_amd/functional.py
@@ -1201,6 +1201,58 @@
 
 
 @_on_operand_device
+def se_squeeze(partial, batch, hw, w_reduce, b_reduce, out=None):
+    if partial.dim() != 2 or partial.shape[0] % batch:
+        raise ValueError(f'partial has shape {tuple(partial.shape)}, expected (B C, nblk) with B = {batch}')
+    c, csq = partial.shape[0] // batch, w_reduce.shape[0]
+    if w_reduce.numel() != csq * c or b_reduce.numel() != csq:
+        raise ValueError(f'w_reduce / b_reduce have {w_reduce.numel()} / {b_reduce.numel()} entries, expected {csq * c} / {csq}')
+    if out is None:
+        out = torch.empty(batch, csq, device=partial.device, dtype=torch.float32)
+    elif tuple(out.shape) != (batch, csq):
+        raise ValueError(f'out has shape {tuple(out.shape)}, expected {(batch, csq)}')
+    _hip.run.hs_se_squeeze_fwd(_hip.dev_ptr(partial, 'partial'), batch, c, partial.shape[1], 1.0 / float(hw), _hip.dev_ptr(w_reduce, 'w_reduce'),
+                               _hip.dev_ptr(b_reduce, 'b_reduce'), csq, _hip.dev_ptr(out, 'out'), _hip.stream_ptr())
+    return out
+
+
+def gemm_split_excite_route(channels, c_squeezed, c_out, pixels, aligned=True):
+    r = _route(_hip.lib.hs_gemm_split_excite_route(channels, c_squeezed, c_out, pixels, int(bool(aligned))), 'hs_gemm_split_excite_route')
+    return None if r is None else f'ks{r >> 4}_w{r & 15}'
+
+
+@_on_operand_device
+def gemm_split_excite(sw, x, squeezed, w_expand_t, b_expand, shift=None, act=ACT_NONE, residual=None, out=None, gate_out=None):
+    b, cin, h, w = x.shape
+    if cin != sw.c_in:
+        raise ValueError(f'input has {cin} channels, the weight {sw.c_in}')
+    shape = (b, sw.c_out, h, w)
+    if out is None:
+        out = torch.empty(shape, device=x.device, dtype=torch.float32)
+    elif tuple(out.shape) != shape:
+        raise ValueError(f'out has shape {tuple(out.shape)}, expected {shape}')
+    if residual is not None and tuple(residual.shape) != shape:
+        raise ValueError(f'residual has shape {tuple(residual.shape)}, expected {shape}')
+    if shift is not None and shift.numel() != sw.c_out:
+        raise ValueError(f'shift has {shift.numel()} entries, expected {sw.c_out}')
+    if squeezed.dim() != 2 or squeezed.shape[0] != b:
+        raise ValueError(f'squeezed has shape {tuple(squeezed.shape)}, expected ({b}, Csq)')
+    csq = squeezed.shape[1]
+    if tuple(w_expand_t.shape) != (csq, cin) or b_expand.numel() != cin:
+        raise ValueError(f'w_expand_t has shape {tuple(w_expand_t.shape)} and b_expand {b_expand.numel()} entries, expected {(csq, cin)} and {cin}')
+    if gate_out is not None and tuple(gate_out.shape) != (b, cin):
+        raise ValueError(f'gate_out has shape {tuple(gate_out.shape)}, expected {(b, cin)}')
+    _hip.run.hs_gemm_split_excite_fwd(_hip.dev_ptr(sw.frag, 'w_frag', torch.float16), _hip.dev_ptr(sw.inv, 'w_inv'),
+                                      _hip.dev_ptr(squeezed, 'squeezed'), csq, _hip.dev_ptr(w_expand_t, 'w_expand_t'),
+                                      _hip.dev_ptr(b_expand, 'b_expand'), _hip.dev_ptr(x, 'x'),
+                                      _hip.dev_ptr(shift, 'shift') if shift is not None else None, int(act),
+                                      _hip.dev_ptr(residual, 'residual') if residual is not None else None,
+                                      _hip.dev_ptr(out, 'out'), b, sw.c_out, cin, sw.kp, h * w,
+                                      _hip.dev_ptr(gate_out, 'gate_out') if gate_out is not None else None, _hip.stream_ptr())
+    return out
+
+
+@_on_operand_device
 def gemm_split_conv2x2(sw, x, shift=None, act=ACT_NONE, out=None, pool_partial=None):
     b, cin, h, w = x.shape
     if 4 * cin != sw.c_in:
diff --git a/hyperseg_amd/utils/inference.py b/hyperseg_amd/utils/inference.py
--- a/hyperseg_amd/utils/inference.py
+++ b/hyperseg_amd/utils/inference.py
@@ -219,6 +219,7 @@
 STEM_DW = os.environ.get('HS_STEM_DW', '1') != '0'
 HS_GEMM_SE = os.environ.get('HS_GEMM_SE', '1') != '0'
 GEMM_SE_MAX_CIN = 512
+GEMM_EXCITE_MAX_CIN = 0
 FUSE_EXPAND_MIN_PIXELS = int(os.environ.get('HS_FUSE_EXPAND_MIN_PIXELS', '2048'))
 FUSE_EXPAND_MAX_CIN = int(os.environ.get('HS_FUSE_EXPAND_MAX_CIN', '40'))
 
@@ -436,13 +437,24 @@
             if sw is not None:
                 if (HS_GEMM_SE and y.is_cuda and not gated and cmid <= GEMM_SE_MAX_CIN and
                         HF.gemm_split_se_route(cmid, pooled.shape[1], self._red_w.shape[0], sw.c_out, ho * wo,
-                                               aligned=(pooled.data_ptr() | red.weight.data_ptr()) % 16 == 0) is not None):
+                                               aligned=(pooled.data_ptr() | red.weight.data_ptr() | self._exp_t.data_ptr()) % 16 == 0) is not None):
                     se_ops = (pooled, ho * wo, red.weight, red.bias, self._exp_t, exp.bias)
                     if self.defer_shift:
                         if skip is None:
                             return HF.gemm_split_se(sw, y, *se_ops)
                         return HF.gemm_split_se(sw, y, *se_ops, residual=skip, out=skip)
                     return HF.gemm_split_se(sw, y, *se_ops, shift=proj.shift, residual=skip)
+                if (HS_GEMM_SE and y.is_cuda and not gated and cmid <= GEMM_EXCITE_MAX_CIN and
+                        HF.se_gate_route(cmid, pooled.shape[1], self._red_w.shape[0],
+                                         aligned=(pooled.data_ptr() | red.weight.data_ptr()) % 16 == 0) == 'two_launch' and
+                        HF.gemm_split_excite_route(cmid, self._red_w.shape[0], sw.c_out, ho * wo,
+                                                   aligned=self._exp_t.data_ptr() % 16 == 0) is not None):
+                    ex_ops = (HF.se_squeeze(pooled, b, ho * wo, red.weight, red.bias), self._exp_t, exp.bias)
+                    if self.defer_shift:
+                        if skip is None:
+                            return HF.gemm_split_excite(sw, y, *ex_ops)
+                        return HF.gemm_split_excite(sw, y, *ex_ops, residual=skip, out=skip)
+                    return HF.gemm_split_excite(sw, y, *ex_ops, shift=proj.shift, residual=skip)
                 gate = se_gate()
                 if self.defer_shift:
                     if skip is None:
diff --git a/include/hyperseg_hip.h b/include/hyperseg_hip.h
--- a/include/hyperseg_hip.h
+++ b/include/hyperseg_hip.h
@@ -416,6 +416,13 @@
                          float* y, int32_t batch, int32_t c_out, int32_t c_in, int32_t kp, int32_t pixels,
                          float* gate_out, float* squeezed_out, void* stream);
 int hs_gemm_split_se_route(int32_t channels, int32_t nblk, int32_t c_squeezed, int32_t c_out, int32_t pixels, int32_t aligned16);
+int hs_gemm_split_excite_fwd(const void* w_frag, const float* w_inv, const float* squeezed, int32_t c_squeezed,
+                             const float* w_expand_t, const float* b_expand, const float* x, const float* shift, int32_t act,
+                             const float* residual, float* y, int32_t batch, int32_t c_out, int32_t c_in, int32_t kp,
+                             int32_t pixels, float* gate_out, void* stream);
+int hs_gemm_split_excite_route(int32_t channels, int32_t c_squeezed, int32_t c_out, int32_t pixels, int32_t aligned16);
+int hs_se_squeeze_fwd(const float* partial, int32_t batch, int32_t channels, int32_t nblk, float inv_hw, const float* w_reduce,
+                      const float* b_reduce, int32_t c_squeezed, float* squeezed, void* stream);
 int hs_gemm_split_conv2x2_fwd(const void* w_frag, const float* w_inv, const float* x, const float* shift, int32_t act, float* y,
                               float* pool_partial, int32_t batch, int32_t c_out, int32_t c_in, int32_t kp, int32_t Ho,
                               int32_t Wo, void* stream);
```
